# brown-ivl/manus

Hardware: AMD Instinct MI355X
Metric: train iters/sec (fwd+bwd) 300k Gaussians @1080p, 8 views; PSNR parity (higher is better)
Workload: dtype f32

## Files before the change

### include/manus_hip.h

```cpp
#ifndef MANUS_HIP_H
#define MANUS_HIP_H

#include <stddef.h>
#include <stdint.h>

#ifdef __cplusplus
extern "C" {
#endif

#define MGR_VERSION 100
#define MGR_CAM_FLOATS 40
#define MGR_TILE 16
#define MGR_MAX_BONES 32

enum {
    MGR_OK = 0,
    MGR_EINVAL = -1,
    MGR_ENOMEM = -2,
    MGR_EHIP = -3,
    MGR_EOVERFLOW = -4,
    MGR_ECUT = -6,
    MGR_ETIER = -7,
    MGR_ESTATE = -8
};
// ... 235 lines not shown
int mgr_fk_adam(int U, int J, const int32_t* frames_listed, const float* d_theta, float* theta, float* m, float* v,
                const float* mask, const float* lo, const float* hi, double lr_rot, double lr_trans, double beta1, double beta2,
                double eps, int step, void* stream);

#define MGR_FK_MAX_KEYPOINTS 64
size_t mgr_fk_terms_workspace_bytes(int U, int J, int K);
int mgr_fk_backward_terms(int V, int J, int F, int U, const int32_t* frames_listed, const int32_t* view_rows,
                          const int32_t* frame_of_view, const float* rest, const float* local, const int32_t* parents, const float* base,
                          const float* theta, const float* mask, const float* d_transforms, float* d_theta,
                          const float* theta_ref, const int32_t* neighbours,
                          double w_dev_rot, double w_smooth_rot, double w_dev_trans, double w_smooth_trans,
                          int K, const int32_t* kp_bone, const float* kp_offset, const float* kp_target, const float* kp_weight, double w_kp,
                          double* values, void* workspace, size_t workspace_bytes, void* stream);

size_t mgr_fk_terms2d_workspace_bytes(int U, int J, int K, int C);
int mgr_fk_backward_terms2d(int V, int J, int F, int U, const int32_t* frames_listed, const int32_t* view_rows,
                            const int32_t* frame_of_view, const float* rest, const float* local, const int32_t* parents, const float* base,
                            const float* theta, const float* mask, const float* d_transforms, float* d_theta,
                            const float* theta_ref, const int32_t* neighbours,
                            double w_dev_rot, double w_smooth_rot, double w_dev_trans, double w_smooth_trans,
                            int K, const int32_t* kp_bone, const float* kp_offset, const float* kp_target, const float* kp_weight, double w_kp,
                            int C, const float* kp2d_proj, const float* kp2d_target, const float* kp2d_weight,
                            double w_kp2d, double delta, double z_min, float* kp2d_dist,
                            double* values, void* workspace, size_t workspace_bytes, void* stream);

#define MGR_TRI_MAX_CAMERAS 64
int mgr_triangulate(int F, int C, int K, const float* proj, const float* targets, const float* weights,
                    double tau, double min_conf, int min_views, double z_min, double det_min,
                    int refit_rounds, int gn_iters,
                    float* xyz, float* conf, int32_t* n_inliers, uint8_t* inliers, float* dist, void* stream);

int mgr_project_points(int N, const float* xyz, const float* K9, const float* E12, float* uv,
                       void* stream);

int mgr_dilate_mask(int H, int W, int kernel_size, const uint8_t* mask, uint8_t* scratch, uint8_t* out,
                    void* stream);
int mgr_points_outside_mask(int N, const float* xyz, const float* K9, const float* E12, int H, int W,
                            const uint8_t* mask, int n_keypoints, const float* keypoints, uint8_t* out,
                            void* stream);
int mgr_keypoint_far_mask(int N, const float* xyz, int n_keypoints, const float* keypoints, float thresh,
                          uint8_t* out, void* stream);

size_t mgr_knn3_workspace_bytes(int N);
int mgr_knn3_mean_dist2(int N, const float* xyz, float* out, void* workspace,
                        size_t workspace_bytes, void* stream);

#define MGR_KNN_MAX_K 512
#ifndef MGR_KNN_CELL_K_DIV
#define MGR_KNN_CELL_K_DIV 16.0f
#endif
#define MGR_KNN_CELL_MIN_POINTS 2.0f
size_t mgr_knn_self_workspace_bytes(int N, int k);
int mgr_knn_self(int N, const float* xyz, int k, int include_self, float* out_d2, int32_t* out_idx, float* out_sigma,
                 int32_t* out_count, void* workspace, size_t workspace_bytes, void* stream);

#define MGR_LOOP_LAMBDA 1.0f
#define MGR_LOOP_SQRT2 1.41421356237309505f
size_t mgr_outlier_scores_workspace_bytes(int N, int k);
int mgr_outlier_scores(int N, const float* xyz, int k, int include_self, float prob, float* out_score, uint8_t* out_mask,
                       float* out_sigma, float* out_plof, double* out_stats, void* workspace, size_t workspace_bytes,
                       void* stream);

int mgr_l1_loss_grad(int64_t count, const float* a, const float* b, float scale, float* dL_da,
                     float* loss_sum, void* stream);

size_t mgr_image_loss_workspace_bytes(int V, int H, int W);
int mgr_image_loss(int V, int H, int W, const float* pred, const float* target, float w_l1, float w_ssim,
                   float grad_scale, float loss_offset, float* dL_dpred, float* sums, void* workspace,
                   size_t workspace_bytes, void* stream);
int mgr_image_loss_tiles(int V, int H, int W, const float* pred, const float* target, const float* bg3,
                         const uint32_t* tile_start, float w_l1, float w_ssim, float grad_scale, float loss_offset,
                         float* dL_dpred, float* sums, void* workspace, size_t workspace_bytes, void* stream);
int mgr_image_loss_tiles_list(int V, int H, int W, const float* target, const float* bg3, const uint32_t* tile_start,
                              void* workspace, size_t workspace_bytes, void* stream);
size_t mgr_image_loss_target_map_words(int V, int H, int W);
int mgr_image_loss_target_map(int V, int H, int W, const float* target, const float* bg3, uint32_t* map, void* stream);
int mgr_image_loss_tiles_list_mapped(int V, int H, int W, const uint32_t* map, const float* bg3, const uint32_t* tile_start,
                                     void* workspace, size_t workspace_bytes, int workspace_kept, void* stream);
int mgr_views_forward_attach_loss_list(const void* raster_workspace, int V, int H, int W, const uint32_t* map,
                                       void* loss_workspace, size_t loss_workspace_bytes);
int mgr_image_loss_tiles_finish(int V, int H, int W, const float* pred, const float* target, float w_l1, float w_ssim,
                                float grad_scale, float loss_offset, float* dL_dpred, float* sums, void* workspace,
                                size_t workspace_bytes, void* stream);

#define MGR_IL2D_DENSE 1
size_t mgr_image_loss2d_workspace_bytes(int V, int H, int W);
int mgr_image_loss2d_block(void);
int mgr_image_loss2d(int V, int H, int W, const float* pred, const float* target, const float* mask, float w_l1, float w_ssim,
                     float grad_scale, float loss_offset, float* dL_dpred, float* sums, float* view_sums, int flags,
                     void* workspace, size_t workspace_bytes, void* stream);

size_t mgr_map_loss_workspace_bytes(int V, int H, int W);
int mgr_map_loss(int V, int H, int W, const float* alpha, const float* mask, const float* depth, const float* depth_target,
                 float w_mask, float w_depth, float grad_scale, float* dL_dalpha, float* dL_ddepth, float* sums,
                 void* workspace, size_t workspace_bytes, void* stream);

int mgr_exposure_block(void);
size_t mgr_exposure_workspace_bytes(int V, int H, int W);
int mgr_exposure_apply(int V, int H, int W, int C, const int32_t* cam_of_view, const float* E, const float* img, float* out,
                       void* stream);
int mgr_exposure_backward(int V, int H, int W, int C, const int32_t* cam_of_view, const float* E, const float* img,
                          const float* g_in, float* g_out, float* dE, void* workspace, size_t workspace_bytes, void* stream);
int mgr_exposure_adam(int C, int U, const int32_t* cams_listed, int V, const int32_t* cam_of_view, const float* dE, float* E,
                      float* m, float* v, double lr, double beta1, double beta2, double eps, int step, void* stream);

size_t mgr_lpips_net_bytes(int net);
int mgr_lpips_net_pack(int net, const float* const* conv_w, const float* const* conv_b, const float* const* lin_w, void* blob,
                       size_t blob_bytes, void* stream);
size_t mgr_lpips_workspace_bytes(int net, int H, int W, int need_grad);
int mgr_lpips_layout(int net, int H, int W, int need_grad, size_t* offsets, int n);
int mgr_lpips(int net, int V, int H, int W, const float* pred, const float* target, const float* mask, const void* blob,
              size_t blob_bytes, int normalize, float grad_scale, float* values, float* dL_dpred, int accumulate,
              void* workspace, size_t workspace_bytes, void* stream);
size_t mgr_lpips_conv_scratch_bytes(int Cin, int Cout, int KH, int KW);
int mgr_lpips_conv(int Cin, int Cout, int H, int W, int KH, int KW, int stride, int pad, const float* x, const float* gate,
                   const float* w, const float* bias, int relu, int transposed, float* y, void* scratch, size_t scratch_bytes,
                   void* stream);
enum { MGR_LPIPS_F32 = 0, MGR_LPIPS_BF16 = 1 };
size_t mgr_lpips_net_bytes_op(int net, int operands);
int mgr_lpips_net_pack_op(int net, const float* const* conv_w, const float* const* conv_b, const float* const* lin_w, void* blob,
                          size_t blob_bytes, void* stream, int operands);
int mgr_lpips_op(int net, int V, int H, int W, const float* pred, const float* target, const float* mask, const void* blob,
                 size_t blob_bytes, int normalize, float grad_scale, float* values, float* dL_dpred, int accumulate,
                 void* workspace, size_t workspace_bytes, void* stream, int operands);
size_t mgr_lpips_conv_scratch_bytes_op(int Cin, int Cout, int KH, int KW, int operands);
int mgr_lpips_conv_op(int Cin, int Cout, int H, int W, int KH, int KW, int stride, int pad, const float* x, const float* gate,
                      const float* w, const float* bias, int relu, int transposed, float* y, void* scratch, size_t scratch_bytes,
                      void* stream, int operands);

size_t mgr_lpips_roi_workspace_bytes(int net, int V, const int* rects, int need_grad);
size_t mgr_lpips_taps_bytes(int net, int h, int w);
int mgr_lpips_roi_taps_op(int net, int H, int W, const int* rect, const float* target_v, const float* mask_v, const void* blob,
                          size_t blob_bytes, int normalize, float* taps_out, void* workspace, size_t workspace_bytes, void* stream,
                          int operands);
int mgr_lpips_roi_op(int net, int V, int H, int W, const int* rects, const float* pred, const float* target, const float* mask,
                     const void* blob, size_t blob_bytes, int normalize, const float* grad_scales, float* values, float* dL_dpred,
                     int accumulate, const float* const* target_taps, void* workspace, size_t workspace_bytes, void* stream,
                     int operands);
int mgr_lpips_roi(int net, int V, int H, int W, const int* rects, const float* pred, const float* target, const float* mask,
                  const void* blob, size_t blob_bytes, int normalize, const float* grad_scales, float* values, float* dL_dpred,
                  int accumulate, const float* const* target_taps, void* workspace, size_t workspace_bytes, void* stream);

#define LP_MAX_BATCH 16
size_t mgr_lpips_roi_batch_workspace_bytes(int net, int V, const int* rects, int need_grad, int max_batch);
int mgr_lpips_roi_taps_batch_op(int net, int V, int H, int W, const int* rects, const float* target, const float* mask, const void* blob,
                                size_t blob_bytes, int normalize, float* const* taps_out, int max_batch, void* workspace,
                                size_t workspace_bytes, void* stream, int operands);
int mgr_lpips_roi_batch_op(int net, int V, int H, int W, const int* rects, const float* pred, const float* target, const float* mask,
                           const void* blob, size_t blob_bytes, int normalize, const float* grad_scales, float* values, float* dL_dpred,
                           int accumulate, const float* const* target_taps, void* workspace, size_t workspace_bytes, void* stream,
                           int operands, int max_batch);
int mgr_lpips_roi_batch(int net, int V, int H, int W, const int* rects, const float* pred, const float* target, const float* mask,
                        const void* blob, size_t blob_bytes, int normalize, const float* grad_scales, float* values, float* dL_dpred,
                        int accumulate, const float* const* target_taps, void* workspace, size_t workspace_bytes, void* stream,
                        int max_batch);

enum { MGR_LPIPS_STORE_F32 = 0, MGR_LPIPS_STORE_BF16 = 1 };
size_t mgr_lpips_workspace_bytes_st(int net, int H, int W, int need_grad, int storage);
int mgr_lpips_layout_st(int net, int H, int W, int need_grad, size_t* offsets, int n, int storage);
size_t mgr_lpips_taps_bytes_st(int net, int h, int w, int storage);
size_t mgr_lpips_roi_batch_workspace_bytes_st(int net, int V, const int* rects, int need_grad, int max_batch, int storage);
int mgr_lpips_st(int net, int V, int H, int W, const float* pred, const float* target, const float* mask, const void* blob,
                 size_t blob_bytes, int normalize, float grad_scale, float* values, float* dL_dpred, int accumulate, void* workspace,
                 size_t workspace_bytes, void* stream, int operands, int storage);
int mgr_lpips_roi_batch_st(int net, int V, int H, int W, const int* rects, const float* pred, const float* target, const float* mask,
                           const void* blob, size_t blob_bytes, int normalize, const float* grad_scales, float* values, float* dL_dpred,
// ... 105 lines not shown
```

### manus_amd/_lib.py

```python
import ctypes
import os

import weakref

import torch

_HERE = os.path.dirname(os.path.abspath(__file__))
_VARIANT = os.environ.get("MANUS_HIP_VARIANT", "")
LIB_PATH = os.path.join(_HERE, "libmanus_hip%s.so" % ("_" + _VARIANT if _VARIANT else ""))
_LIB = None

MGR_CAM_FLOATS = 40
MGR_MAX_BONES = 32
MGR_FK_MAX_KEYPOINTS = 64
MGR_TRI_MAX_CAMERAS = 64
MGR_FRAMES_MAX_VIEWS = 16

MGR_OK, MGR_EINVAL, MGR_ENOMEM, MGR_EHIP, MGR_EOVERFLOW, MGR_ECUT, MGR_ETIER, MGR_ESTATE = 0, -1, -2, -3, -4, -6, -7, -8
MGR_FWD_CHECK, MGR_FWD_NO_BLEND, MGR_FWD_BLEND_ONLY, MGR_FWD_DEPTH_CUT = 1, 2, 4, 8
MGR_FWD_SKIP_BOX_LARGE, MGR_FWD_SKIP_BOX_MID, MGR_FWD_SKIP_SORT_BEHIND, MGR_FWD_RANK_LARGE = 16, 32, 128, 256
MGR_FWD_IMAGE_KEPT, MGR_FWD_REPAIR, MGR_FWD_SPREAD = 1024, 2048, 4096
MGR_BWD_CHECK, MGR_BWD_OUTPUTS_KEPT = 1, 512
MGR_OVF_PAIRS, MGR_OVF_CUT, MGR_OVF_TIER, MGR_OVF_FLAGS_MASK, MGR_OVF_REPAIRED_SHIFT = 1, 2, 4, 0xFFFF, 16
MGR_TIERS_BOX_LARGE, MGR_TIERS_BOX_MID, MGR_TIERS_WIDE_RECT = 1, 2, 4
MGR_TIERS_NEAR_SMALL_SHIFT, MGR_TIERS_NEAR_LARGE_SHIFT, MGR_TIERS_NEAR_MASK = 8, 16, 0xFF
MGR_TIERS_BEYOND_SMALL_SHIFT, MGR_TIERS_BEYOND_SMALL_MASK = 24, 0x7F
MGR_LPIPS_F32, MGR_LPIPS_BF16 = 0, 1
MGR_LPIPS_STORE_F32, MGR_LPIPS_STORE_BF16 = 0, 1
MGR_IL2D_DENSE = 1
MGR_KNN_MAX_K = 512
LP_MAX_BATCH = 16

c_int, c_i64, c_f32, c_vp, c_sz = ctypes.c_int, ctypes.c_int64, ctypes.c_float, ctypes.c_void_p, ctypes.c_size_t


class MgrFrameView(ctypes.Structure):
    _fields_ = [("offset", ctypes.c_int64), ("x0", ctypes.c_int32), ("y0", ctypes.c_int32), ("x1", ctypes.c_int32), ("y1", ctypes.c_int32),
                ("rx0", ctypes.c_int32), ("ry0", ctypes.c_int32), ("rx1", ctypes.c_int32), ("ry1", ctypes.c_int32),
                ("bg", ctypes.c_float * 3), ("slot", ctypes.c_int32)]


SIGNATURES = {
    "mgr_version": (c_int, []),
    "mgr_build_variant": (c_int, []),
    "mgr_raster_repair_max_tiles": (c_int, []),
    "mgr_last_error": (ctypes.c_char_p, []),
    "mgr_raster_workspace_bytes": (c_sz, [c_int, c_int, c_int, c_int, c_i64]),
    "mgr_raster_forward": (c_int, [c_int, c_int, c_int, c_int, c_vp, c_vp, c_vp, c_i64, c_vp, c_i64, c_vp,
                                   c_i64, c_vp, c_i64, c_vp, c_vp, c_vp, c_sz, c_i64, c_int, c_vp]),
    "mgr_raster_backward": (c_int, [c_int, c_int, c_int, c_int, c_vp, c_vp, c_vp, c_i64, c_vp, c_i64, c_vp,
                                    c_i64, c_vp, c_i64, c_vp, c_vp, c_vp, c_vp, c_vp, c_vp, c_vp, c_vp, c_sz,
                                    c_i64, c_int, c_vp]),
    "mgr_raster_blend_features": (c_int, [c_int, c_int, c_int, c_int, c_int, c_vp, c_i64, c_vp, c_int, c_vp, c_vp, c_vp, c_sz,
                                          c_i64, c_vp]),
    "mgr_raster_feat_backward_workspace_bytes": (c_sz, [c_int, c_int, c_int, c_int, c_int, c_i64]),
    "mgr_raster_blend_features_backward": (c_int, [c_int] * 5 + [c_vp, c_vp, c_i64, c_vp, c_i64, c_vp, c_i64, c_vp, c_int] + [c_vp] * 9
                                           + [c_vp, c_sz, c_i64, c_vp, c_sz, c_int, c_vp]),
    "mgr_raster_forward_seq_sync": (c_int, [c_vp, ctypes.POINTER(ctypes.c_uint32), c_vp]),
    "mgr_sh_to_half": (c_int, [c_int, c_vp, c_vp, c_vp]),
    "mgr_views_forward": (c_int, [c_int] * 7 + [c_vp] * 12 + [c_vp, c_sz, c_i64, c_int, c_vp]),
    "mgr_views_backward": (c_int, [c_int] * 7 + [c_vp] * 13 + [c_f32] + [c_vp] * 10 + [c_vp, c_sz, c_i64, c_int, c_vp]),
    "mgr_views_pose_workspace_bytes": (c_sz, [c_int, c_int, c_int]),
    "mgr_views_backward_pose": (c_int, [c_int] * 7 + [c_vp] * 13 + [c_f32] + [c_vp] * 10 + [c_vp, c_sz, c_i64, c_int, c_vp, c_vp, c_sz,
                                        c_vp]),
    "mgr_views_maps_backward_workspace_bytes": (c_sz, [c_int, c_int, c_int, c_int, c_i64]),
    "mgr_views_maps_backward": (c_int, [c_int] * 6 + [c_vp] * 11 + [c_int] + [c_vp] * 5 + [c_vp, c_sz, c_i64, c_vp, c_sz, c_int, c_vp]),
    "mgr_views_maps_pose_workspace_bytes": (c_sz, [c_int, c_int, c_int]),
    "mgr_views_maps_backward_pose": (c_int, [c_int] * 6 + [c_vp] * 11 + [c_int] + [c_vp] * 5 + [c_vp, c_sz, c_i64, c_vp, c_sz, c_int] +
                                     [c_int, c_vp, c_vp, c_sz, c_vp]),
    "mgr_raster_record_bytes": (c_int, []),
    "mgr_raster_layout": (c_int, [c_int, c_int, c_int, c_int, c_i64, ctypes.POINTER(c_sz), c_int]),
    "mgr_raster_status_sync": (c_int, [c_vp, ctypes.POINTER(c_i64), ctypes.POINTER(ctypes.c_int32), c_vp]),
    "mgr_raster_set_status_mirror": (c_int, [c_vp, c_vp]),
    "mgr_raster_set_cut_margin": (c_int, [c_f32, c_int, c_f32, c_f32, c_int]),
    "mgr_raster_set_cut_penalty": (c_int, [c_int]),
    "mgr_raster_status_tiers_sync": (c_int, [c_vp, ctypes.POINTER(c_i64), ctypes.POINTER(ctypes.c_int32),
                                             ctypes.POINTER(ctypes.c_int32), c_vp]),
    "mgr_debug_pair_alpha": (c_int, [c_int, c_vp, c_vp, c_vp, c_vp, c_vp, c_vp]),
    "mgr_raster_debug_binning_sync": (c_int, [c_vp, c_int, c_int, c_int, c_int, c_i64, c_int, c_vp, c_vp,
                                              c_i64, c_vp]),
    "mgr_skin_weights_fwd": (c_int, [c_int, c_vp, c_vp, c_int, c_int, c_int, c_int, c_int, c_vp, c_vp, c_vp,
                                     c_vp]),
    "mgr_skin_weights_bwd": (c_int, [c_int, c_vp, c_vp, c_int, c_int, c_int, c_int, c_int, c_vp, c_vp, c_vp,
                                     c_vp, c_int, c_vp]),
    "mgr_skin_weights_bwd_indexed": (c_int, [c_int, c_vp, c_vp, c_int, c_int, c_int, c_int, c_int, c_vp, c_vp, c_vp,
                                             c_vp, c_vp, c_vp, c_int, c_vp]),
    "mgr_skin_grid_bwd_workspace_bytes": (c_sz, [c_int, c_int, c_int, c_int]),
    "mgr_skin_grid_bwd": (c_int, [c_int, c_vp, c_vp, c_int, c_int, c_int, c_int, c_int, c_vp, c_vp, c_vp, c_vp, c_vp, c_int,
                                  c_vp, c_vp, c_vp, c_int, c_vp, c_sz, c_vp]),
    "mgr_skin_grid_adam": (c_int, [c_vp, c_vp, c_vp, c_int, c_vp, c_int, c_int, c_vp, c_vp, ctypes.c_double, ctypes.c_double, ctypes.c_double,
                                   ctypes.c_double, c_int, c_int, c_f32, c_vp]),
    "mgr_skin_grid_refine_workspace_bytes": (c_sz, [c_int]),
    "mgr_skin_grid_refine": (c_int, [c_vp, c_vp, c_vp, c_int, c_vp, c_vp, c_int, c_int, c_vp, c_vp, ctypes.c_double, ctypes.c_double,
                                     ctypes.c_double, ctypes.c_double, c_int, c_int, c_f32, ctypes.c_double, c_int, c_f32, c_vp, c_vp,
                                     c_sz, c_vp]),
    "mgr_skin_rows_mask": (c_int, [c_int, c_int, c_vp, c_vp, c_vp]),
    "mgr_views_backward_run_lists": (c_int, [c_int]),
    "mgr_views_active_list": (c_int, [c_vp, c_int, c_int, c_int, c_int, c_i64, ctypes.POINTER(c_vp), ctypes.POINTER(c_vp)]),
    "mgr_lbs_cov_fwd": (c_int, [c_int, c_int, c_int, c_vp, c_vp, c_vp, c_vp, c_vp, c_vp, c_vp, c_vp, c_vp]),
    "mgr_lbs_cov_bwd": (c_int, [c_int, c_int, c_int, c_vp, c_vp, c_vp, c_vp, c_vp, c_vp, c_vp, c_vp, c_vp,
                                c_vp, c_vp, c_vp, c_vp]),
    "mgr_lbs_cov_fwd_rows": (c_int, [c_int, c_int, c_int, c_vp, c_vp, c_vp, c_vp, c_vp, c_vp, c_vp, c_vp, c_int, c_vp]),
    "mgr_lbs_cov_bwd_rows": (c_int, [c_int, c_int, c_int, c_vp, c_vp, c_vp, c_vp, c_vp, c_vp, c_vp, c_vp, c_int, c_vp,
                                     c_vp, c_vp, c_vp, c_vp]),
    "mgr_lbs_pose_workspace_bytes": (c_sz, [c_int, c_int, c_int]),
    "mgr_lbs_pose_bwd": (c_int, [c_int, c_int, c_int, c_vp, c_vp, c_vp, c_vp, c_vp, c_vp, c_vp, c_vp, c_int, c_vp, c_vp, c_sz, c_vp]),
    "mgr_sh_color_fwd_rows": (c_int, [c_int, c_int, c_vp, c_vp, c_i64, c_vp, c_i64, c_int, c_vp, c_vp, c_vp]),
    "mgr_sh_color_bwd_rows": (c_int, [c_int, c_int, c_vp, c_vp, c_i64, c_vp, c_i64, c_int, c_vp, c_vp, c_vp, c_vp, c_vp,
                                      c_vp]),
    "mgr_sh_color_fwd": (c_int, [c_int, c_int, c_vp, c_vp, c_i64, c_vp, c_i64, c_vp, c_vp, c_vp]),
    "mgr_sh_color_bwd": (c_int, [c_int, c_int, c_vp, c_vp, c_i64, c_vp, c_i64, c_vp, c_vp, c_vp, c_vp, c_vp,
                                 c_vp]),
    "mgr_pack_camera": (c_int, [c_f32, c_f32, c_vp, c_vp, c_vp, c_vp, c_vp]),
    "mgr_bone_transforms": (c_int, [c_int, c_int, c_vp, c_vp, c_vp, c_vp]),
    "mgr_pose_apply": (c_int, [c_int, c_int, c_int] + [c_vp] * 8 + [c_vp]),
    "mgr_pose_backward": (c_int, [c_int, c_int, c_int, c_int] + [c_vp] * 10 + [c_vp]),
    "mgr_pose_adam": (c_int, [c_int, c_int] + [c_vp] * 9 + [ctypes.c_double] * 5 + [c_int, c_vp]),
    "mgr_pose_prior_workspace_bytes": (c_sz, [c_int, c_int]),
    "mgr_pose_backward_prior": (c_int, [c_int, c_int, c_int, c_int] + [c_vp] * 10 + [c_vp] + [ctypes.c_double] * 4 + [c_vp, c_vp, c_sz, c_vp]),
    "mgr_fk_apply": (c_int, [c_int, c_int, c_int] + [c_vp] * 11 + [c_vp]),
    "mgr_fk_backward": (c_int, [c_int, c_int, c_int, c_int] + [c_vp] * 11 + [c_vp]),
    "mgr_fk_adam": (c_int, [c_int, c_int] + [c_vp] * 8 + [ctypes.c_double] * 5 + [c_int, c_vp]),
    "mgr_fk_terms_workspace_bytes": (c_sz, [c_int, c_int, c_int]),
    "mgr_fk_backward_terms": (c_int, [c_int, c_int, c_int, c_int] + [c_vp] * 11 + [c_vp, c_vp] + [ctypes.c_double] * 4
                              + [c_int] + [c_vp] * 4 + [ctypes.c_double] + [c_vp, c_vp, c_sz, c_vp]),
    "mgr_fk_terms2d_workspace_bytes": (c_sz, [c_int, c_int, c_int, c_int]),
    "mgr_fk_backward_terms2d": (c_int, [c_int, c_int, c_int, c_int] + [c_vp] * 11 + [c_vp, c_vp] + [ctypes.c_double] * 4
                                + [c_int] + [c_vp] * 4 + [ctypes.c_double] + [c_int] + [c_vp] * 3 + [ctypes.c_double] * 3 + [c_vp]
                                + [c_vp, c_vp, c_sz, c_vp]),
    "mgr_triangulate": (c_int, [c_int, c_int, c_int, c_vp, c_vp, c_vp, ctypes.c_double, ctypes.c_double, c_int, ctypes.c_double,
                                ctypes.c_double, c_int, c_int] + [c_vp] * 5 + [c_vp]),
    "mgr_project_points": (c_int, [c_int, c_vp, c_vp, c_vp, c_vp, c_vp]),
    "mgr_dilate_mask": (c_int, [c_int, c_int, c_int, c_vp, c_vp, c_vp, c_vp]),
    "mgr_points_outside_mask": (c_int, [c_int, c_vp, c_vp, c_vp, c_int, c_int, c_vp, c_int, c_vp, c_vp, c_vp]),
    "mgr_keypoint_far_mask": (c_int, [c_int, c_vp, c_int, c_vp, c_f32, c_vp, c_vp]),
    "mgr_knn3_workspace_bytes": (c_sz, [c_int]),
    "mgr_knn3_mean_dist2": (c_int, [c_int, c_vp, c_vp, c_vp, c_sz, c_vp]),
    "mgr_knn_self_workspace_bytes": (c_sz, [c_int, c_int]),
    "mgr_knn_self": (c_int, [c_int, c_vp, c_int, c_int, c_vp, c_vp, c_vp, c_vp, c_vp, c_sz, c_vp]),
    "mgr_outlier_scores_workspace_bytes": (c_sz, [c_int, c_int]),
    "mgr_outlier_scores": (c_int, [c_int, c_vp, c_int, c_int, c_f32, c_vp, c_vp, c_vp, c_vp, c_vp, c_vp, c_sz, c_vp]),
    "mgr_exchange_mask": (c_int, [c_int, c_vp, c_int, ctypes.POINTER(c_i64), ctypes.POINTER(c_int), c_i64, c_vp, c_vp, c_vp, c_vp]),
    "mgr_exchange_index_workspace_bytes": (c_sz, [c_int]),
    "mgr_exchange_index": (c_int, [c_int, c_vp, c_vp, c_vp, c_vp, c_sz, c_vp]),
    "mgr_exchange_pack": (c_int, [c_int, c_int, c_vp, c_vp, c_int, ctypes.POINTER(c_i64), ctypes.POINTER(c_int), c_i64, c_vp, c_vp]),
    "mgr_exchange_unpack": (c_int, [c_int, c_int, c_vp, c_vp, c_int, ctypes.POINTER(c_i64), ctypes.POINTER(c_int), c_i64, c_vp, c_vp,
                                    c_i64, c_vp]),
    "mgr_exchange_pack_rows": (c_int, [c_int, c_int, c_vp, c_vp, c_vp, c_int, ctypes.POINTER(c_i64), ctypes.POINTER(c_int), c_i64, c_vp, c_vp]),
    "mgr_exchange_unpack_rows": (c_int, [c_int, c_int, c_vp, c_vp, c_vp, c_int, ctypes.POINTER(c_i64), ctypes.POINTER(c_int), c_i64, c_vp, c_vp,
                                         c_i64, c_vp]),
    "mgr_l1_loss_grad": (c_int, [c_i64, c_vp, c_vp, c_f32, c_vp, c_vp, c_vp]),
    "mgr_image_loss_workspace_bytes": (c_sz, [c_int, c_int, c_int]),
    "mgr_image_loss": (c_int, [c_int, c_int, c_int, c_vp, c_vp, c_f32, c_f32, c_f32, c_f32, c_vp, c_vp, c_vp, c_sz, c_vp]),
    "mgr_image_loss_tiles": (c_int, [c_int, c_int, c_int, c_vp, c_vp, c_vp, c_vp, c_f32, c_f32, c_f32, c_f32, c_vp, c_vp, c_vp, c_sz,
                                     c_vp]),
    "mgr_image_loss_target_map_words": (c_sz, [c_int, c_int, c_int]),
# ... 216 lines not shown
```

### manus_amd/csrc/image_loss.hip

```cpp
#include "mgr_common.h"
#include "il_list.h"
#include <cstdlib>

#define IL_ACC_SLOTS 64
#define IL_NX (IL_ND + 2 * IL_H1)

struct IlWindow {
    float g[11];
};

typedef mgr_v2f v2f;
__device__ __forceinline__ v2f il_v2(float a) { v2f r = {a, a}; return r; }

__global__ __launch_bounds__(IL_T) void k_image_loss(int H, int W, const float* __restrict__ pred,
                                                     const float* __restrict__ target, IlWindow win, float w_l1,
                                                     float w_ssim, float grad_scale, float* __restrict__ dL_dpred,
                                                     float2* __restrict__ partial, const uint32_t* __restrict__ work_list,
                                                     const uint32_t* __restrict__ work_count, int gxb, int gyb,
                                                     unsigned long long* __restrict__ acc_slots, uint32_t nb, float sum_lim,
                                                     uint32_t* __restrict__ bad_flag) {
    __shared__ v2f s_mix[5][3][IL_NX];
    __shared__ float s_red[4];
    const int tid = threadIdx.x;
    const uint32_t n_work = min(*work_count, nb);
// ... 312 lines not shown
        if (!tile_start) return;
    }
    uint32_t my_rank[(ILS_MAXW / IL_W + ILS_T) / ILS_T];
    int nmine = 0;
    for (int b = tid; b < gxb; b += ILS_T, ++nmine) {
        const int lo = max(b * IL_W - 2 * IL_H1, 0), hi = min(b * IL_W + IL_ND, W);
        uint32_t any = ((s_cand[b >> 5] >> (b & 31)) & 1u) ? 0u : 1u;
        for (int k = lo >> 5; k <= (hi - 1) >> 5 && !any; ++k) {
            uint32_t m = s_diff[k];
            const int base = k << 5;
            if (lo > base) m &= ~0u << (lo - base);
            if (hi < base + 32) m &= ~0u >> (base + 32 - hi);
            any |= m;
        }
        my_rank[nmine] = any ? atomicAdd(&s_n, 1u) : 0xFFFFFFFFu;
        if (!any) {
            const uint32_t bid = ((uint32_t)v * gridDim.x + blockIdx.x) * (uint32_t)gxb + (uint32_t)b;
            const int wcnt = min((b + 1) * IL_W, W) - b * IL_W;
            partial[bid] = make_float2(0.f, (float)(wcnt * 3 * rows));
        }
    }
    __syncthreads();
    if (tid == 0 && s_n) s_base = atomicAdd(work_count, s_n);
    __syncthreads();
    nmine = 0;
    for (int b = tid; b < gxb; b += ILS_T, ++nmine)
        if (my_rank[nmine] != 0xFFFFFFFFu)
            work_list[s_base + my_rank[nmine]] = ((uint32_t)v * gridDim.x + blockIdx.x) * (uint32_t)gxb + (uint32_t)b;
}

__global__ __launch_bounds__(ILS_T) void k_image_loss_list_mapped(IlListArgs a) {
    __shared__ uint32_t s2[2];
    il_list_mapped_block(a, (int)blockIdx.x, (int)blockIdx.y, s2);
}

__global__ __launch_bounds__(IL_ACC_SLOTS) void k_image_loss_fold(unsigned long long* __restrict__ acc_slots, long long total_px3,
                                                                  float* __restrict__ sums, float ca, float cb, float cc,
                                                                  uint32_t* __restrict__ work_count) {
    __shared__ unsigned long long s_fin[3 * IL_ACC_SLOTS];
    const int tid = threadIdx.x;
#pragma unroll
    for (int q = 0; q < 3; ++q) {
        s_fin[q * IL_ACC_SLOTS + tid] = acc_slots[3 * tid + q];
        acc_slots[3 * tid + q] = 0ull;
    }
    __syncthreads();
    if (tid == 0) {
        long long t_l1 = 0, t_ss = 0;
        unsigned long long t_px = 0;
        for (int k = 0; k < IL_ACC_SLOTS; ++k) {
            t_l1 += (long long)s_fin[k];
            t_ss += (long long)s_fin[IL_ACC_SLOTS + k];
            t_px += s_fin[2 * IL_ACC_SLOTS + k];
        }
        const double ta = (double)t_l1 * (1.0 / 4294967296.0);
        const double tb = (double)t_ss * (1.0 / 4294967296.0) + (double)((unsigned long long)total_px3 - t_px);
        const bool bad = work_count[1] != 0u;
        const float qnan = __int_as_float(0x7FC00000);
        sums[0] = bad ? qnan : (float)ta;
        sums[1] = bad ? qnan : (float)tb;
        sums[2] = bad ? qnan : (float)((double)ca * ta + (double)cb * tb + (double)cc);
        work_count[0] = 0u;
        work_count[1] = 0u;
    }
}


static size_t il_slots_offset(int64_t nb) { return (((size_t)nb * (sizeof(float2) + sizeof(uint32_t)) + 256) + 63) & ~(size_t)63; }
extern "C" size_t mgr_image_loss_workspace_bytes(int V, int H, int W) {
    if (V <= 0 || H <= 0 || W <= 0) return 0;
    return il_slots_offset(il_blocks(V, H, W)) + 3 * IL_ACC_SLOTS * sizeof(unsigned long long);
}

static int image_loss_impl(int V, int H, int W, const float* pred, const float* target, const float* bg3,
                           const uint32_t* tile_start, float w_l1, float w_ssim, float grad_scale, float loss_offset,
                           float* dL_dpred, float* sums, void* workspace, size_t workspace_bytes, void* stream_, int phase = 0,
                           const uint32_t* tmap = nullptr, bool clean = false) {
    if (V <= 0 || H <= 0 || W <= 0) return mgr_fail(MGR_EINVAL, "mgr_image_loss: bad sizes");
    if ((!target && !(phase == 1 && tmap)) || !workspace || (phase != 1 && (!pred || !dL_dpred || !sums))) return mgr_fail(MGR_EINVAL, "mgr_image_loss: null pointer");
    if (H > 65535 || V > 65535) return mgr_fail(MGR_EINVAL, "mgr_image_loss: H and V must fit a grid dimension");
    if (workspace_bytes < mgr_image_loss_workspace_bytes(V, H, W))
        return mgr_fail(MGR_ENOMEM, "mgr_image_loss: workspace too small");
    hipStream_t stream = (hipStream_t)stream_;
    IlWindow win;
    float sum = 0.f;
    for (int i = 0; i < 11; ++i) {
        win.g[i] = (float)exp(-(double)((i - 5) * (i - 5)) / (2.0 * 1.5 * 1.5));
        sum += win.g[i];
    }
    for (int i = 0; i < 11; ++i) win.g[i] /= sum;
    const dim3 grid((W + IL_W - 1) / IL_W, (H + 1) / 2, V);
    const int64_t nb = il_blocks(V, H, W);
    if (nb >= (1ll << 32)) return mgr_fail(MGR_EINVAL, "mgr_image_loss: image batch too large");
    float2* partial = (float2*)workspace;
    uint32_t* work_list = (uint32_t*)((char*)workspace + (size_t)nb * sizeof(float2));
    uint32_t* work_count = (uint32_t*)((char*)workspace + (size_t)nb * (sizeof(float2) + sizeof(uint32_t)) + 64);
    if (W > ILS_MAXW) return mgr_fail(MGR_EINVAL, "mgr_image_loss: image wider than 16384");
    unsigned long long* acc_slots = (unsigned long long*)((char*)workspace + il_slots_offset(nb));
    if (phase != 2 && !clean)
        MGR_HIP(hipMemsetAsync(work_count, 0, (size_t)((char*)(acc_slots + 3 * IL_ACC_SLOTS) - (char*)work_count), stream));
    if (phase == 2) {
    } else if (tile_start && tmap) {
        MGR_PROF("k_image_loss_list", stream);
        const IlListArgs la = il_list_args(V, H, W, tmap, tile_start, workspace);
        hipLaunchKernelGGL(k_image_loss_list_mapped, dim3((unsigned)la.nbx, V), dim3(ILS_T), 0, stream, la);
    } else if (tile_start) {
        MGR_PROF("k_image_loss_list", stream);
        hipLaunchKernelGGL(k_image_loss_list, dim3(grid.y, V), dim3(ILS_T), 0, stream, H, W, (int)grid.x, target, bg3, tile_start,
                           partial, work_list, work_count, tmap, (uint32_t*)nullptr);
    } else {
        MGR_PROF("k_image_loss_scan", stream);
        hipLaunchKernelGGL(k_image_loss_scan, dim3(grid.y, V), dim3(ILS_T), 0, stream, H, W, (int)grid.x, pred, target, dL_dpred,
                           partial, work_list, work_count);
    }
    if (phase == 1) return MGR_OK;
    {
        MGR_PROF("k_image_loss", stream);
#ifndef IL_GRID
#define IL_GRID (256 * 5)
#endif
        const int64_t pb = nb < IL_GRID ? nb : IL_GRID;
        const float sum_lim = (float)(2147483648.0 * (1.0 - 1.0 / 1048576.0) / (double)nb);
        hipLaunchKernelGGL(k_image_loss, dim3((unsigned)pb), dim3(IL_T), 0, stream, H, W, pred, target, win, w_l1, w_ssim,
                           grad_scale, dL_dpred, partial, (const uint32_t*)work_list, (const uint32_t*)work_count,
                           (int)grid.x, (int)grid.y, acc_slots, (uint32_t)nb, sum_lim, work_count + 1);
    }
    hipLaunchKernelGGL(k_image_loss_fold, dim3(1), dim3(IL_ACC_SLOTS), 0, stream, acc_slots, (long long)V * H * W * 3,
                       sums, grad_scale * w_l1, -grad_scale * w_ssim, loss_offset, work_count);
    MGR_LAUNCH_CHECK("k_image_loss", stream, 0);
    return MGR_OK;
}

extern "C" int mgr_image_loss(int V, int H, int W, const float* pred, const float* target, float w_l1, float w_ssim,
                              float grad_scale, float loss_offset, float* dL_dpred, float* sums, void* workspace,
                              size_t workspace_bytes, void* stream_) {
    return image_loss_impl(V, H, W, pred, target, nullptr, nullptr, w_l1, w_ssim, grad_scale, loss_offset, dL_dpred, sums,
                           workspace, workspace_bytes, stream_);
}

extern "C" int mgr_image_loss_tiles(int V, int H, int W, const float* pred, const float* target, const float* bg3,
                                    const uint32_t* tile_start, float w_l1, float w_ssim, float grad_scale, float loss_offset,
                                    float* dL_dpred, float* sums, void* workspace, size_t workspace_bytes, void* stream_) {
    if (!bg3 || !tile_start) return mgr_fail(MGR_EINVAL, "mgr_image_loss_tiles: null pointer");
    return image_loss_impl(V, H, W, pred, target, bg3, tile_start, w_l1, w_ssim, grad_scale, loss_offset, dL_dpred, sums,
                           workspace, workspace_bytes, stream_);
}

extern "C" int mgr_image_loss_tiles_list(int V, int H, int W, const float* target, const float* bg3, const uint32_t* tile_start,
                                         void* workspace, size_t workspace_bytes, void* stream_) {
    if (!bg3 || !tile_start) return mgr_fail(MGR_EINVAL, "mgr_image_loss_tiles_list: null pointer");
    return image_loss_impl(V, H, W, nullptr, target, bg3, tile_start, 0.f, 0.f, 0.f, 0.f, nullptr, nullptr, workspace,
                           workspace_bytes, stream_, 1);
}

extern "C" int mgr_image_loss_tiles_finish(int V, int H, int W, const float* pred, const float* target, float w_l1, float w_ssim,
                                           float grad_scale, float loss_offset, float* dL_dpred, float* sums, void* workspace,
                                           size_t workspace_bytes, void* stream_) {
    return image_loss_impl(V, H, W, pred, target, nullptr, nullptr, w_l1, w_ssim, grad_scale, loss_offset, dL_dpred, sums,
                           workspace, workspace_bytes, stream_, 2);
}

extern "C" size_t mgr_image_loss_target_map_words(int V, int H, int W) {
    if (V <= 0 || H <= 0 || W <= 0) return 0;
    return (size_t)V * ((H + 1) / 2) * ((W + 31) / 32);
}

extern "C" int mgr_image_loss_target_map(int V, int H, int W, const float* target, const float* bg3, uint32_t* map, void* stream_) {
    if (V <= 0 || H <= 0 || W <= 0) return mgr_fail(MGR_EINVAL, "mgr_image_loss_target_map: bad sizes");
    if (!target || !bg3 || !map) return mgr_fail(MGR_EINVAL, "mgr_image_loss_target_map: null pointer");
    if (H > 65535 || V > 65535 || W > ILS_MAXW) return mgr_fail(MGR_EINVAL, "mgr_image_loss_target_map: image too large");
    hipLaunchKernelGGL(k_image_loss_list, dim3((H + 1) / 2, V), dim3(ILS_T), 0, (hipStream_t)stream_, H, W, (W + IL_W - 1) / IL_W,
                       target, bg3, (const uint32_t*)nullptr, (float2*)nullptr, (uint32_t*)nullptr, (uint32_t*)nullptr,
                       (const uint32_t*)nullptr, map);
    MGR_LAUNCH_CHECK("k_image_loss_list", (hipStream_t)stream_, 0);
    return MGR_OK;
}

extern "C" int mgr_image_loss_tiles_list_mapped(int V, int H, int W, const uint32_t* map, const float* bg3, const uint32_t* tile_start,
                                                void* workspace, size_t workspace_bytes, int workspace_kept, void* stream_) {
    if (!map || !bg3 || !tile_start) return mgr_fail(MGR_EINVAL, "mgr_image_loss_tiles_list_mapped: null pointer");
    return image_loss_impl(V, H, W, nullptr, nullptr, bg3, tile_start, 0.f, 0.f, 0.f, 0.f, nullptr, nullptr, workspace,
                           workspace_bytes, stream_, 1, map, workspace_kept != 0);
}
```

### manus_amd/csrc/mgr_common.h

```cpp
#pragma once
#include <hip/hip_runtime.h>
#include <stdint.h>
#include <stdio.h>
#include <string.h>

#include "../../include/manus_hip.h"

#define MGR_WAVE 64

extern thread_local char g_mgr_err[512];

static inline int mgr_fail(int code, const char* fmt, const char* a = "", const char* b = "") {
    snprintf(g_mgr_err, sizeof(g_mgr_err), fmt, a, b);
    return code;
}

#define MGR_HIP(call)                                                                      \
    do {                                                                                   \
        hipError_t e_ = (call);                                                            \
        if (e_ != hipSuccess) return mgr_fail(MGR_EHIP, "%s: %s", #call, hipGetErrorString(e_)); \
    } while (0)

#define MGR_LAUNCH_CHECK(name, stream, debug)                                              \
    do {                                                                                   \
        hipError_t e_ = hipGetLastError();                                                 \
        if (e_ != hipSuccess) return mgr_fail(MGR_EHIP, "launch %s: %s", name, hipGetErrorString(e_)); \
        if (debug) {                                                                       \
            e_ = hipStreamSynchronize(stream);                                             \
            if (e_ != hipSuccess) return mgr_fail(MGR_EHIP, "sync %s: %s", name, hipGetErrorString(e_)); \
        }                                                                                  \
    } while (0)

void mgr_prof_begin(const char* name, hipStream_t stream);
void mgr_prof_end(hipStream_t stream);
extern int g_mgr_prof_on;
bool mgr_prof_match(const char* name);
struct MgrProfScope {
    hipStream_t s;
    bool on;
    MgrProfScope(const char* name, hipStream_t stream) : s(stream), on(g_mgr_prof_on != 0 && mgr_prof_match(name)) {
        if (on) mgr_prof_begin(name, s);
    }
    ~MgrProfScope() {
        if (on) mgr_prof_end(s);
    }
};
#define MGR_PROF(name, stream) MgrProfScope mgr_prof_scope_(name, stream)

#define MGR_WHY_UNITS 1u
#define MGR_WHY_VIEW_TILES 2u
#define MGR_WHY_CAND 4u
#define MGR_WHY_LIST 8u
#define MGR_WHY_EMPTY 16u
#define MGR_WHY_WINDOW 32u
#define MGR_REP_CAND 8192
#define MGR_REP_TARGET 3072
#define MGR_REP_VIEW_TILES 256
#define MGR_REP_MAX_TILES 65536
struct __attribute__((aligned(16))) MgrRepUnit {
    uint32_t vt, quad, nlist, start;
    uint32_t ck0, done_lo, done_hi, ntail;
    uint32_t ov_start, ov_ck0, p0, ck_first;
    uint32_t beyond;
    uint32_t pad[3];
};
struct __attribute__((aligned(16))) MgrRepTile {
    uint32_t tile, unit, zc, zw;
};
struct MgrRepView {
    uint32_t n, x0, y0, x1, y1, pad[3];
    MgrRepTile t[MGR_REP_VIEW_TILES];
};
struct MgrRep {
    MgrRepUnit* unit;
    float4* state;
    uint32_t* last;
    uint32_t* cnt;
    uint32_t* tile_rep;
    unsigned long long* cand;
    MgrRepView* view;
    uint32_t max_units, list_cap, ck_cap, list_base, ck_base;
};
struct MgrHeader {
    uint32_t total_pairs;
    uint32_t overflow;
    uint32_t epoch;
    uint32_t queue_len;
    uint32_t queue_head;
    uint32_t queue_head2;
    uint32_t n_items;
    uint32_t item_head;
    uint32_t queue_small;
    uint32_t queue_head3;
    uint32_t n_active;
    uint32_t queue_len_i;
    uint32_t acc_pairs, acc_flags;
    uint32_t tiers;
    uint32_t sort_big;
    uint32_t n_runs[4];
    uint32_t bwd_seq, rows_seq, rows_pending;
    uint32_t rows_owner[2];
    uint32_t fwd_seq, img_seq, img_owner[2], img_bg[3];
    uint32_t n_rep_units, rep_list_used, rep_ck_used;
    uint32_t rep_why;
    MgrRep rep;
    uint32_t sort_huge;
    uint32_t sort_large;
    uint32_t sort_near_large;
    uint32_t feat_seq, feat_dims[5], feat_flags;
    uint32_t spare[45 - 7 - sizeof(MgrRep) / 4];
    uint32_t queue_giant;
    uint32_t n_groups;
    uint32_t split_head, group_head;
    uint32_t pad2[56 - 8 - 68 + 64 - 4];
    uint32_t qctr[16 * 64];
    uint32_t qctr_f[16 * 64];
};
#define MGR_NCTR 16
#define MGR_HOLE 0xFFFFFFFEu
#define MGR_FEAT_CUT 1u
struct MgrFeatStamp {
    uint32_t dims[5], flags;
};
#define MGR_SKIP_BOX_LARGE 1
#define MGR_SKIP_BOX_MID 2
#define MGR_SKIP_SORT_BEHIND 4
#define MGR_SKIP_RANK_LARGE 8

#ifndef MGR_GREC_BYTES
#define MGR_GREC_BYTES 64
// ... 428 lines not shown
```

### manus_amd/csrc/raster_bwd.hip

```cpp
#include <atomic>

#include "instance_math.h"

#ifdef MGR_STATS
__device__ unsigned long long g_stats[16];
extern "C" int mgr_debug_stats(unsigned long long* dst) {
    return (int)hipMemcpyFromSymbol(dst, HIP_SYMBOL(g_stats), sizeof(unsigned long long) * 16);
}
__device__ unsigned long long g_bhist[3][65];
extern "C" int mgr_debug_bhist(unsigned long long* dst) {
    return (int)hipMemcpyFromSymbol(dst, HIP_SYMBOL(g_bhist), sizeof(unsigned long long) * 3 * 65);
}
#define BH(r, c, v) do { const int c_ = (c); const unsigned long long v_ = (unsigned long long)(v); if (lane == 0) atomicAdd(&g_bhist[r][c_], v_); } while (0)
#define MGR_STAT(i, v) do { const unsigned long long v_ = (unsigned long long)(v); if (lane == 0) atomicAdd(&g_stats[i], v_); } while (0)
#else
#define MGR_STAT(i, v)
#endif

#ifdef BWD_PROF
__device__ unsigned long long g_bprof[8];
extern "C" int mgr_debug_bprof(unsigned long long* dst) {
    return (int)hipMemcpyFromSymbol(dst, HIP_SYMBOL(g_bprof), sizeof(unsigned long long) * 8);
}
#define BP(k) { const long long now_ = wall_clock64(); acc_[k] += now_ - tp_; tp_ = now_; }
// ... 983 lines not shown
    inst_bwd_body<2, BMAX, MIXED, SH_HALF, true, NVV, POSE>(blk, n2, active_list + 2 * (size_t)N, MGR_IB_ARGS, pose_valid);
}
template <int NVV, int BMAX, bool MIXED, bool SH_HALF>
__global__ __launch_bounds__(IB_THREADS) __attribute__((amdgpu_waves_per_eu(MGR_IB_WAVES, MGR_IB_WAVES))) void k_inst_bwd_runs(MGR_IB_PARAMS) {
    inst_bwd_runs<NVV, BMAX, MIXED, SH_HALF, false>(MGR_IB_ALL, nullptr);
}

template <int G, int BMAX, bool MIXED, bool SH_HALF>
__global__ __launch_bounds__(IB_THREADS) __attribute__((amdgpu_waves_per_eu(MGR_IB_WAVES, MGR_IB_WAVES))) void k_inst_bwd_pose(MGR_IB_PARAMS, unsigned char* __restrict__ pose_valid) {
    inst_bwd_body<G, BMAX, MIXED, SH_HALF, false, 8, true>((int)blockIdx.x, (int)hdr->n_active, active_list, MGR_IB_ARGS, pose_valid);
}
template <int NVV, int BMAX, bool MIXED, bool SH_HALF>
__global__ __launch_bounds__(IB_THREADS) __attribute__((amdgpu_waves_per_eu(MGR_IB_WAVES, MGR_IB_WAVES))) void k_inst_bwd_runs_pose(MGR_IB_PARAMS, unsigned char* __restrict__ pose_valid) {
    inst_bwd_runs<NVV, BMAX, MIXED, SH_HALF, true>(MGR_IB_ALL, pose_valid);
}

template <int NV>
__global__ __launch_bounds__(256) void k_pose_part_views(int n_art, int B, int n_chunks, const float4* __restrict__ iacc,
                                                         const unsigned char* __restrict__ valid,
                                                         const float* __restrict__ skin_w, float* __restrict__ part) {
    constexpr int IPB = 256 / NV;
    __shared__ float s_rec[256 * MGR_POSE_REC];
    __shared__ unsigned char s_lst[NV * 256];
    __shared__ int s_cnt[8], s_wc[8 * 4];
    const int tid = threadIdx.x, vl = tid & (NV - 1), il = tid / NV;
    float pacc[12];
#pragma unroll
    for (int k = 0; k < 12; ++k) pacc[k] = 0.f;
    for (int c = blockIdx.x; c < n_chunks; c += gridDim.x) {
        const int i = c * IPB + il;
        const bool on = i < n_art && valid[(size_t)i * NV + vl] != 0;
        if (on) {
            const float4* o = iacc + ((size_t)i * NV + vl) * 3;
            const float4 a = o[0], b = o[1], d = o[2];
            float* r = s_rec + tid * MGR_POSE_REC;
            r[0] = a.x; r[1] = a.y; r[2] = a.z; r[3] = a.w; r[4] = b.x; r[5] = b.y; r[6] = b.z; r[7] = b.w;
            r[8] = d.x; r[9] = d.y; r[10] = d.z; r[11] = d.w;
            r[12] = __int_as_float(i);
        }
        pose_wg_lists<256>(tid, NV, on ? vl : -1, s_lst, s_cnt, s_wc);
        pose_wg_accumulate<256>(tid, NV, B, s_rec, s_lst, s_cnt, skin_w, pacc);
        __syncthreads();
    }
    pose_wg_store<256>(tid, NV, B, s_rec, pacc, part + (size_t)blockIdx.x * NV * B * 12);
}

static std::atomic<int> g_inst_runs{[] { const char* e = getenv("MANUS_INST_RUNS"); return e ? atoi(e) : 1; }()};
extern "C" int mgr_views_backward_run_lists(int on) { return g_inst_runs.exchange(on); }

struct CanonGrads {
    int B, n_art, sh_half;
    const float *xyz, *log_scale, *rot, *op_logit, *f_dc, *f_rest, *skin_w, *transforms;
    const int32_t* radii;
    float grad2d_scale;
    float *d_xyz, *d_ls, *d_rot, *d_op, *d_fdc, *d_frest, *d_w, *st_grad2d, *st_vis;
    int32_t* st_radii;
    float *d_T, *pose_part;
};

static int pose_view_slots(int n_art, int Gv) {
    const int ipb = 256 / Gv, chunks = (n_art + ipb - 1) / ipb;
    return chunks < MGR_POSE_MAX_WG ? chunks : MGR_POSE_MAX_WG;
}
static size_t pose_part_bytes(int N, int B, int Gv) { return ((size_t)pose_view_slots(N, Gv) * Gv * B * 12 * sizeof(float) + 255) & ~(size_t)255; }
extern "C" size_t mgr_views_pose_workspace_bytes(int V, int N, int B) {
    if (V <= 0 || N <= 0 || B <= 0) return 0;
    const int Gv = V <= 1 ? 1 : V <= 2 ? 2 : V <= 4 ? 4 : 8;
    return pose_part_bytes(N, B, Gv) + (size_t)N * Gv;
}

static int raster_backward_impl(int V, int N, int W, int H, const float* cams, const float* bg,
                                   const float* means3D, int64_t s_means, const float* cov3D,
                                   int64_t s_cov, const float* colors, int64_t s_col,
                                   const float* opacity, int64_t s_op, const float* out_color,
                                   const float* dL_dcolor, float* dL_dmeans3D, float* dL_dmeans2D, float* dL_dcolors,
                                   float* dL_dopacity, float* dL_dcov3D, const CanonGrads* canon, void* workspace,
                                   size_t workspace_bytes, int64_t cap, int flags, void* stream_) {
    (void)colors; (void)s_col; (void)opacity; (void)s_op;
    hipStream_t stream = (hipStream_t)stream_;
    if (V <= 0 || N < 0 || W <= 0 || H <= 0 || cap < 0)
        return mgr_fail(MGR_EINVAL, "mgr_raster_backward: bad sizes");
    if (!cams || !bg || !dL_dcolor || !out_color || !workspace)
        return mgr_fail(MGR_EINVAL, "mgr_raster_backward: null pointer");
    if (N == 0) return MGR_OK;
    if (!canon && (!means3D || !cov3D || !dL_dmeans3D || !dL_dmeans2D || !dL_dcolors || !dL_dopacity || !dL_dcov3D))
        return mgr_fail(MGR_EINVAL, "mgr_raster_backward: null pointer");
    const int gx = (W + 15) / 16, gy = (H + 15) / 16;
    const MgrLayout L = mgr_layout(V, N, W, H, cap);
    if (workspace_bytes < L.total) return mgr_fail(MGR_ENOMEM, "mgr_raster_backward: workspace too small");
    char* ws = (char*)workspace;
    MgrHeader* hdr = (MgrHeader*)(ws + L.header);
    static std::atomic<uint32_t> g_epoch{0};
    uint32_t epoch = g_epoch.fetch_add(1) + 1;
    if (epoch == 0) epoch = g_epoch.fetch_add(1) + 1;

    { MGR_PROF("k_blend_bwd", stream); hipLaunchKernelGGL(k_blend_bwd, dim3(256 * BWD_WAVES), dim3(256), 0, stream, N, W, H, gx, gy,
                       (const uint32_t*)(ws + L.sorted_gid), (const MgrGRec*)(ws + L.grec), (const uint32_t*)(ws + L.n_contrib),
                       (const float4*)(ws + L.ckpt), (const uint4*)(ws + L.items), hdr, out_color,
                       dL_dcolor, (uint32_t*)(ws + L.pair_tag), (float4*)(ws + L.pair_grad),
                       (uint32_t*)(ws + L.inst_tag), (uint32_t)cap, epoch); }
    MGR_LAUNCH_CHECK("k_blend_bwd", stream, flags & MGR_BWD_CHECK);
    if (canon) {
        const int Gv = V <= 1 ? 1 : V <= 2 ? 2 : V <= 4 ? 4 : 8;
        const int ipb = 256 / Gv;
        const size_t lds = (size_t)Gv * (MGR_CAM_FLOATS + (canon->skin_w ? IB_TSTRIDE(canon->B) : 0)) * sizeof(float);
        float4* iacc = (float4*)(ws + L.inst_grad);
        uint32_t* alist = (uint32_t*)(ws + L.inst_grad + (size_t)N * Gv * 48);
        const int ipb2 = IB_THREADS / Gv;
        const bool mixed = canon->skin_w && canon->n_art < N;
        int rounds = (int)((long long)N / ((long long)ipb * 1024));
        rounds = rounds < 1 ? 1 : (rounds > IG_ROUNDS ? IG_ROUNDS : rounds);
        const dim3 grid((N + ipb2 - 1) / ipb2), grid_g((N + ipb * rounds - 1) / (ipb * rounds));
        for (int v0 = 0; v0 < V; v0 += Gv) {
            const int vc = V - v0 < Gv ? V - v0 : Gv;
            const int accm = v0 > 0 ? 1 : 0;
            if (v0 > 0) {
                MGR_HIP(hipMemsetAsync(&hdr->n_active, 0, 4, stream));
                MGR_HIP(hipMemsetAsync(&hdr->n_runs[0], 0, 12, stream));
            }
            const bool runs = g_inst_runs.load(std::memory_order_relaxed) != 0 && Gv >= 4 && canon->B <= 24 && N < (1 << 24);
            const int rounds_r = rounds < Gv ? rounds : Gv;
            const dim3 grid_gr((N + ipb * rounds_r - 1) / (ipb * rounds_r));
            uint32_t* rlist = alist + (size_t)N;
            unsigned char* row_state = V <= Gv ? (unsigned char*)(rlist + 3 * (size_t)N) : nullptr;
            const int kept = (flags & MGR_BWD_OUTPUTS_KEPT) && V <= Gv ? 1 : 0;
#define MGR_IG_LAUNCH(GG)                                                                                             \
    hipLaunchKernelGGL((k_inst_gather<GG>), grid_g, dim3(256), 0, stream, v0, vc, N, canon->B, canon->n_art, canon->radii, \
                       (const ushort4*)(ws + L.rect), (const uint32_t*)(ws + L.pair_off),                             \
                       (const uint32_t*)(ws + L.pair_tag), (const float4*)(ws + L.pair_grad),                        \
                       (const uint32_t*)(ws + L.inst_tag), (uint32_t)cap, epoch, accm, rounds, iacc, alist, hdr, canon->d_xyz, canon->d_ls, canon->d_rot, canon->d_op, canon->d_fdc,    \
                       canon->d_frest, canon->d_w, canon->st_grad2d, canon->st_vis, canon->st_radii, runs && GG == 8 ? rlist : (uint32_t*)nullptr)
#define MGR_IB_LAUNCH(GG, BB)                                                                                         \
    if (mixed && canon->sh_half) MGR_IB_LAUNCH2(GG, BB, true, true);                                                  \
    else if (mixed) MGR_IB_LAUNCH2(GG, BB, true, false);                                                              \
    else if (canon->sh_half) MGR_IB_LAUNCH2(GG, BB, false, true);                                                     \
    else MGR_IB_LAUNCH2(GG, BB, false, false)
#define MGR_IB_LAUNCH2(GG, BB, MX, HF)                                                                                \
    hipLaunchKernelGGL((k_inst_bwd<GG, BB, MX, HF>), grid, dim3(IB_THREADS), lds, stream, v0, vc, N, canon->B, canon->n_art, W, H, cams, canon->xyz, \
                       canon->log_scale, canon->rot, canon->op_logit, canon->f_dc, canon->f_rest, canon->skin_w,      \
                       canon->transforms, (const float4*)iacc, (const uint32_t*)alist, (const MgrHeader*)hdr,         \
                       canon->grad2d_scale, accm, canon->d_xyz, canon->d_ls, canon->d_rot, canon->d_op, canon->d_fdc, \
                       canon->d_frest, canon->d_w, canon->st_grad2d)
            {
                MGR_PROF("k_inst_gather", stream);
#define MGR_IGR_LAUNCH(GG)                                                                                            \
    hipLaunchKernelGGL((k_inst_gather_runs<GG>), grid_gr, dim3(256), 0, stream, v0, vc, N, canon->B, canon->n_art, canon->radii, \
                       (const ushort4*)(ws + L.rect), (const uint32_t*)(ws + L.pair_off),                             \
                       (const uint32_t*)(ws + L.pair_tag), (const float4*)(ws + L.pair_grad),                        \
                       (const uint32_t*)(ws + L.inst_tag), (uint32_t)cap, epoch, accm, rounds_r, iacc, alist, hdr, canon->d_xyz, canon->d_ls, canon->d_rot, canon->d_op, canon->d_fdc, \
                       canon->d_frest, canon->d_w, canon->st_grad2d, canon->st_vis, canon->st_radii, rlist, row_state, kept)
                const bool old_gather = g_inst_runs.load(std::memory_order_relaxed) == 2 && Gv == 8;
                if (runs && !old_gather) {
                    if (Gv == 8) MGR_IGR_LAUNCH(8);
                    else if (Gv == 4) MGR_IGR_LAUNCH(4);
                    else if (Gv == 2) MGR_IGR_LAUNCH(2);
                    else MGR_IGR_LAUNCH(1);
                }
#undef MGR_IGR_LAUNCH
                else if (Gv == 8) MGR_IG_LAUNCH(8);
                else if (Gv == 4) MGR_IG_LAUNCH(4);
                else if (Gv == 2) MGR_IG_LAUNCH(2);
                else MGR_IG_LAUNCH(1);
            }
            MgrProfScope prof_ib(canon->d_T ? "k_inst_bwd_pose" : "k_inst_bwd", stream);
#define MGR_IBR_LAUNCH(MX, HF)                                                                                        \
    if (Gv == 8) MGR_IBR_LAUNCH2(8, MX, HF); else if (Gv == 4) MGR_IBR_LAUNCH2(4, MX, HF); else MGR_IBR_LAUNCH2(2, MX, HF)
// ... 151 lines not shown
```

### manus_amd/csrc/raster_feat.hip

```cpp
#include "instance_math.h"

#define FEAT_MAX_C 32
#define FEAT_GRID 4096

struct FeatArgs {
    int N, W, H, gx, gy, VT;
    uint32_t n_queue, n_busy, cap;
    const uint32_t* tile_queue;
    const uint4* tile_qrec;
    const uint32_t* sorted_gid;
    const MgrGRec* grec;
    const float* depth;
    const float* feat;
    long long s_feat;
    int C, c0, nc;
    int with_z;
    const float* bg;
    float* out;
    int Cout;
    float* out_alpha;
};

template <int CG>
__global__ __launch_bounds__(256) void k_blend_feat(const FeatArgs a) {
// ... 59 lines not shown
                mgr_pair_store(pb, rank & 1, ra.x, ra.y, ra.z, ra.w, rb.x, rb.y, 0.f, 0.f, 0.f, 0u);
                float* fr = frow + rank * CG;
#pragma unroll
                for (int k = 0; k < CG; ++k) fr[k] = f[k];
                if ((cnt & 1) && rank == cnt - 1) {
                    mgr_pair_pad(pb);
#pragma unroll
                    for (int k = 0; k < CG; ++k) fr[CG + k] = 0.0f;
                }
            }
            {
                gid = min(gid_n, gid_max);
                ra = *(const float4*)(gv + gid);
                rb = *((const float4*)(gv + gid) + 1);
                gid_n = sg[min(off + 128u + lane, lastidx)];
            }
            __builtin_amdgcn_wave_barrier();
            const int npair = (cnt + 1) >> 1;
            for (int p = 0; p < npair; ++p) {
                const float4* pp = (const float4*)(slab + p * MGR_PAIR_FLOATS);
                const float4 R0 = pp[0], R1 = pp[1], R2 = pp[2];
                float fa[CG], fb[CG];
                const float* fp = frow + 2 * p * CG;
#pragma unroll
                for (int k = 0; k < CG; ++k) { fa[k] = fp[k]; fb[k] = fp[CG + k]; }
                mgr_v2f dx, dy, G, al;
                bool va, vb;
                mgr_pair_alpha(R0, R1, R2, fpx2, fpy2, dx, dy, G, al, va, vb);
                {
                    const float al_a = (va && !done) ? al.x : 0.0f;
                    const float testT = Tr * (1.0f - al_a);
                    const bool stop = testT < 0.0001f;
                    const float w = stop ? 0.0f : al_a * Tr;
#pragma unroll
                    for (int k = 0; k < CG; ++k) acc[k] += fa[k] * w;
                    Tr = stop ? Tr : testT;
                    done = done || stop;
                }
                {
                    const float al_b = (vb && !done) ? al.y : 0.0f;
                    const float testT = Tr * (1.0f - al_b);
                    const bool stop = testT < 0.0001f;
                    const float w = stop ? 0.0f : al_b * Tr;
#pragma unroll
                    for (int k = 0; k < CG; ++k) acc[k] += fb[k] * w;
                    Tr = stop ? Tr : testT;
                    done = done || stop;
                }
                if (__builtin_amdgcn_ballot_w64(!done) == 0ull) break;
            }
        }
        if (inside) {
            const size_t pix = (size_t)py * W + px;
            if (ns > 0) {
                float* o = a.out + ((size_t)v * a.Cout + a.c0) * P + pix;
#pragma unroll
                for (int k = 0; k < CG; ++k)
                    if (k < ns) o[(size_t)k * P] = acc[k] + Tr * bg_of(k);
            }
            if (a.out_alpha) a.out_alpha[(size_t)v * P + pix] = 1.0f - Tr;
        }
    }
    for (uint32_t q = a.n_busy + blockIdx.x; q < (uint32_t)a.VT; q += gridDim.x) {
        const uint32_t vt = a.tile_queue[q];
        if (vt >= (uint32_t)a.VT) continue;
        const int v = (int)(vt / (uint32_t)T), t = (int)(vt % (uint32_t)T);
        const int px = (t % gx) * 16 + (tid & 15), py = (t / gx) * 16 + (tid >> 4);
        if (px < W && py < H) {
            const size_t pix = (size_t)py * W + px;
            if (ns > 0) {
                float* o = a.out + ((size_t)v * a.Cout + a.c0) * P + pix;
#pragma unroll
                for (int k = 0; k < CG; ++k)
                    if (k < ns) o[(size_t)k * P] = bg_of(k);
            }
            if (a.out_alpha) a.out_alpha[(size_t)v * P + pix] = 0.0f;
        }
    }
}

static int feat_read_state(const char* who, const char* ws, const MgrLayout& L, int V, int N, int W, int H, int64_t cap, int VT,
                           hipStream_t stream, MgrHeader& h) {
    const size_t head_bytes = offsetof(MgrHeader, qctr);
    MGR_HIP(hipMemcpyAsync(&h, ws + L.header, head_bytes, hipMemcpyDeviceToHost, stream));
    MGR_HIP(hipStreamSynchronize(stream));
    if (h.fwd_seq == 0u) return mgr_fail(MGR_ESTATE, "%s: no forward has run on this workspace", who);
    if (h.feat_seq != h.fwd_seq)
        return mgr_fail(MGR_ESTATE, "%s: the last forward on this workspace did not run its blend (MGR_FWD_NO_BLEND)", who);
    if (h.feat_dims[0] != (uint32_t)V || h.feat_dims[1] != (uint32_t)N || h.feat_dims[2] != (uint32_t)W ||
        h.feat_dims[3] != (uint32_t)H || h.feat_dims[4] != (uint32_t)cap)
        return mgr_fail(MGR_ESTATE, "%s: the last forward on this workspace was made for another V, N, W, H or pair capacity", who);
    if (h.feat_flags & MGR_FEAT_CUT)
        return mgr_fail(MGR_ESTATE, "%s: the last forward applied the depth cut (MGR_FWD_DEPTH_CUT): its lists are cut short", who);
    if (h.overflow != 0u)
        return mgr_fail(MGR_ESTATE, "%s: the last forward raised an overflow bit: its lists are incomplete", who);
    if (h.queue_len > (uint32_t)VT || h.queue_len_i > (uint32_t)VT)
        return mgr_fail(MGR_ESTATE, "%s: the header's queue lengths do not fit these sizes", who);
    return MGR_OK;
}

extern "C" int mgr_raster_forward_seq_sync(const void* workspace, uint32_t* seq, void* stream_) {
    hipStream_t stream = (hipStream_t)stream_;
    if (!workspace || !seq) return mgr_fail(MGR_EINVAL, "mgr_raster_forward_seq_sync: null pointer");
    MGR_HIP(hipMemcpyAsync(seq, (const char*)workspace + offsetof(MgrHeader, fwd_seq), 4, hipMemcpyDeviceToHost, stream));
    MGR_HIP(hipStreamSynchronize(stream));
    return MGR_OK;
}

extern "C" int mgr_raster_blend_features(int V, int N, int C, int W, int H, const float* features, int64_t stride_features,
                                         const float* bg_feat, int with_depth, float* out_feat, float* out_alpha,
                                         const void* workspace, size_t workspace_bytes, int64_t cap, void* stream_) {
    hipStream_t stream = (hipStream_t)stream_;
    if (V <= 0 || N < 0 || W <= 0 || H <= 0 || cap < 0 || cap > 0xFFFFFFF0ll)
        return mgr_fail(MGR_EINVAL, "mgr_raster_blend_features: bad sizes");
    if (C < 0 || C > FEAT_MAX_C) return mgr_fail(MGR_EINVAL, "mgr_raster_blend_features: C must be 0 .. 32");
    const int Cout = C + (with_depth ? 1 : 0);
    if (Cout == 0 && !out_alpha) return mgr_fail(MGR_EINVAL, "mgr_raster_blend_features: nothing to render (C = 0, no depth, no alpha)");
    if (!workspace || (Cout > 0 && !out_feat) || (C > 0 && N > 0 && !features))
        return mgr_fail(MGR_EINVAL, "mgr_raster_blend_features: null pointer");
    if (stride_features != 0 && stride_features < (int64_t)N * C)
        return mgr_fail(MGR_EINVAL, "mgr_raster_blend_features: view stride of the features smaller than N * C");
    const int gx = (W + 15) / 16, gy = (H + 15) / 16;
    if (gx > 65535 || gy > 65535) return mgr_fail(MGR_EINVAL, "mgr_raster_blend_features: image too large");
    const MgrLayout L = mgr_layout(V, N, W, H, cap);
    if (workspace_bytes < L.total) return mgr_fail(MGR_ENOMEM, "mgr_raster_blend_features: workspace too small for these sizes");
    const char* ws = (const char*)workspace;
    MgrHeader h;
    const int VT = V * gx * gy;
    {
        const int rc = feat_read_state("mgr_raster_blend_features", ws, L, V, N, W, H, cap, VT, stream, h);
        if (rc != MGR_OK) return rc;
    }

    FeatArgs a;
    a.N = N; a.W = W; a.H = H; a.gx = gx; a.gy = gy; a.VT = VT;
    a.n_queue = h.queue_len_i; a.n_busy = h.queue_len; a.cap = (uint32_t)cap;
    a.tile_queue = (const uint32_t*)(ws + L.tile_queue);
    a.tile_qrec = (const uint4*)(ws + L.tile_qrec);
    a.sorted_gid = (const uint32_t*)(ws + L.sorted_gid);
    a.grec = (const MgrGRec*)(ws + L.grec);
    a.depth = (const float*)(ws + L.depth);
    a.feat = features; a.s_feat = (long long)stride_features; a.C = C;
    a.bg = bg_feat; a.out = out_feat; a.Cout = Cout;
    int c0 = 0;
    bool first = true;
    MGR_PROF("k_blend_feat", stream);
    do {
        const int rem = Cout - c0, g = rem > 4 ? 8 : (rem > 2 ? 4 : 2), n = rem < g ? rem : g;
        a.c0 = c0;
        a.with_z = (with_depth && c0 + n == Cout) ? 1 : 0;
        a.nc = n - a.with_z;
        a.out_alpha = first ? out_alpha : nullptr;
        if (g == 8) hipLaunchKernelGGL(k_blend_feat<8>, dim3(FEAT_GRID), dim3(256), 0, stream, a);
        else if (g == 4) hipLaunchKernelGGL(k_blend_feat<4>, dim3(FEAT_GRID), dim3(256), 0, stream, a);
        else hipLaunchKernelGGL(k_blend_feat<2>, dim3(FEAT_GRID), dim3(256), 0, stream, a);
        MGR_LAUNCH_CHECK("k_blend_feat", stream, 0);
        c0 += n;
        first = false;
    } while (c0 < Cout);
    return MGR_OK;
}

#define FEAT_REC 16
#define FEAT_GEO 8

struct FeatScratch {
    size_t tag, rec, geo, total;
};
static inline FeatScratch feat_scratch_layout(int V, int N, int64_t cap) {
    FeatScratch S;
    const size_t c = (size_t)(cap > 0 ? cap : 1), VN = (size_t)V * (size_t)(N > 0 ? N : 1);
    size_t o = 0;
    S.tag = o; o += mgr_align(c * 4);
    S.rec = o; o += mgr_align(c * FEAT_REC * 4);
    S.geo = o; o += mgr_align(VN * FEAT_GEO * 4);
    S.total = o;
    return S;
}

extern "C" size_t mgr_raster_feat_backward_workspace_bytes(int V, int N, int C, int W, int H, int64_t cap) {
    (void)C; (void)W; (void)H;
    if (V <= 0 || N < 0 || cap < 0) return 0;
    return feat_scratch_layout(V, N, cap).total;
}

struct FeatBwdArgs {
// ... 737 lines not shown
```

### manus_amd/csrc/raster_fwd.hip

```cpp
#include <atomic>
#include <mutex>

#include "instance_math.h"
#include "il_list.h"

#include <cstdlib>
#include <cstring>
#include <map>
#include <string>
#include <vector>

thread_local char g_mgr_err[512] = {0};

int g_mgr_prof_on = 0;
namespace {
struct ProfRec { const char* name; hipEvent_t a, b; };
std::vector<ProfRec> g_prof_recs;
std::vector<hipEvent_t> g_prof_pool;
hipEvent_t prof_event() {
    if (!g_prof_pool.empty()) { hipEvent_t e = g_prof_pool.back(); g_prof_pool.pop_back(); return e; }
    hipEvent_t e;
    if (hipEventCreate(&e) != hipSuccess) return nullptr;
    return e;
}
// ... 1272 lines not shown
#endif
        for (uint32_t p = 0; p < parts; ++p) {
            const uint32_t a = parts == 1u ? lo : st[b0 + p], n = (parts == 1u ? hi : st[b0 + p + 1]) - a;
            if (n == 0) continue;
            __syncthreads();
            if (n <= lds_keys) {
                lds_sort_emit(keys + a, n, s_keys, s_cnt, s_scan, tid, out + a);
            } else {
                uint32_t npad = 1;
                while (npad < n) npad <<= 1;
                bitonic_mirror(keys + a, n, npad, tid, RS_THREADS);
                for (uint32_t t = tid; t < n; t += RS_THREADS) out[a + t] = (uint32_t)keys[a + t];
            }
        }
#ifdef DBS_PROF
        if (tid == 0) {
            const long long t2 = wall_clock64();
            atomicAdd(&g_dbsprof[0], (unsigned long long)(t1 - t0));
            atomicAdd(&g_dbsprof[1], (unsigned long long)(t2 - t1));
            atomicAdd(&g_dbsprof[2], 1ull);
            atomicAdd(&g_dbsprof[3], (unsigned long long)(hi - lo));
            atomicAdd(&g_dbsprof[4], (unsigned long long)parts);
            atomicMax(&g_dbsprof[5], (unsigned long long)(t2 - t0));
            atomicMax(&g_dbsprof[6], (unsigned long long)(hi - lo));
            atomicMax(&g_dbsprof[7], (unsigned long long)(t2 - t_start));
            const uint32_t nk = hi - lo;
            atomicAdd(&g_dbsprof[nk <= 1024u ? 8 : nk <= 2048u ? 9 : nk <= 3072u ? 10 : nk <= 4096u ? 11 : 12], 1ull);
        }
#endif
    }
}

#define DBR_THREADS RS_THREADS
template <int CAP>
__global__ __launch_bounds__(DBR_THREADS) void k_dbin_rank(int N, int V, int items_per_view, const uint32_t* __restrict__ db_start,
                                                           const uint32_t* __restrict__ db_item, const unsigned long long* __restrict__ db_keys,
                                                           uint32_t* __restrict__ db_order, MgrHeader* hdr,
                                                           int no_launch_behind, BgFill fill, int n_sort_blocks) {
    constexpr uint32_t cap_keys = (uint32_t)CAP;
    if ((int)blockIdx.x >= n_sort_blocks) {
        bg_fill_block(fill, hdr, (int)blockIdx.x - n_sort_blocks, (int)gridDim.x - n_sort_blocks);
        return;
    }
    __shared__ __attribute__((aligned(16))) unsigned long long s_keys[CAP];
    __shared__ uint32_t s_cnt[RS_WAVES * 256];
    __shared__ uint32_t s_scan[32];
    const int tid = threadIdx.x;
    const int v = (int)blockIdx.x % V, it = (int)blockIdx.x / V;
    const uint32_t* const ent = db_item + ((size_t)v * items_per_view + it) * 2;
    const uint32_t e0 = ent[0], e1 = ent[1];
    if (e0 == 0u) return;
    const uint32_t* st = db_start + (size_t)v * (MGR_DB_BUCKETS + 1);
    const uint32_t lo = st[~e0], hi = st[e1], n = hi - lo;
    if (n > (uint32_t)MGR_DB_RANK_MAX * 13u / 16u && tid == 0) {
        atomicAdd(&hdr->sort_big, 1u);
        if (n > (uint32_t)MGR_DB_RANK_LARGE * 13u / 16u) atomicAdd(&hdr->sort_near_large, 1u);
        if (n > (uint32_t)MGR_DB_RANK_MAX) atomicAdd(&hdr->sort_large, 1u);
    }
    if (n > cap_keys) {
        if (tid == 0) {
            atomicAdd(&hdr->sort_huge, 1u);
            if (no_launch_behind) atomicOr(&hdr->overflow, MGR_OVF_TIER);
        }
        return;
    }
    lds_sort_emit(db_keys + (size_t)v * N + lo, n, s_keys, s_cnt, s_scan, tid, db_order + (size_t)v * N + lo);
}

#define BIN_SMALL_TILES 2048
__device__ __forceinline__ bool bin_mine(ushort4 box, bool small_variant) {
    const uint32_t tb = (uint32_t)box.z * (uint32_t)box.w;
    return tb > 0u && (tb <= (uint32_t)BIN_SMALL_TILES) == small_variant;
}

#define BCNT_THREADS 256
#define BCNT_PER (MGR_BIN_BLOCK / BCNT_THREADS)
template <bool SMALL>
__global__ __launch_bounds__(BCNT_THREADS) void k_bin_count(int N, int T, int nblk, int bb,
                                                            const uint32_t* __restrict__ db_nvis,
                                                            const ushort4* __restrict__ db_bbox,
                                                            const uint32_t* __restrict__ db_order,
                                                            const ushort4* __restrict__ rect,
                                                            const unsigned long long* __restrict__ alive,
                                                            uint4* __restrict__ db_rec, uint32_t* __restrict__ bin_mat, int xcd_order) {
    extern __shared__ uint32_t s_mem[];
    uint32_t* s_hist = s_mem;
    const int tid = threadIdx.x;
    int v = blockIdx.y, b = blockIdx.x;
    if (xcd_order) {
        const int q = blockIdx.x >> 3;
        v = (blockIdx.x & 7) + 8 * (q / nblk);
        b = q % nblk;
    }
    const ushort4 box = db_bbox[v];
    if (!bin_mine(box, SMALL)) return;
    const uint32_t nvis = db_nvis[v];
    if ((uint32_t)b * (uint32_t)bb >= nvis) return;
    const int TB = (int)box.z * (int)box.w, bw = box.z;
    uint32_t gid[BCNT_PER];
#pragma unroll
    for (int r = 0; r < BCNT_PER; ++r) {
        const uint32_t p = (uint32_t)b * (uint32_t)bb + r * BCNT_THREADS + tid;
        gid[r] = (r * BCNT_THREADS < bb && p < nvis) ? db_order[(size_t)v * N + p] : 0u;
    }
    ushort4 rc[BCNT_PER];
    unsigned long long am[BCNT_PER];
#pragma unroll
    for (int r = 0; r < BCNT_PER; ++r) {
        rc[r] = rect[(size_t)v * N + gid[r]];
        am[r] = alive[(size_t)v * N + gid[r]];
    }
    for (int k = tid; k < TB; k += BCNT_THREADS) s_hist[k] = 0;
    __syncthreads();
#pragma unroll
    for (int r = 0; r < BCNT_PER; ++r) {
        const uint32_t p = (uint32_t)b * (uint32_t)bb + r * BCNT_THREADS + tid;
        if (r * BCNT_THREADS < bb && p < nvis) {
            const uint32_t w = rc[r].z - rc[r].x, h = rc[r].w - rc[r].y;
            db_rec[(size_t)v * N + p] = make_uint4((uint32_t)rc[r].x | ((uint32_t)rc[r].y << 16), w | (h << 16), (uint32_t)am[r],
                                                   (uint32_t)(am[r] >> 32));
            const int org = ((int)rc[r].y - (int)box.y) * bw + (int)rc[r].x - (int)box.x;
            if (w * h <= 64u) {
                const float rw = __frcp_rn((float)max(w, 1u));
                unsigned long long m = am[r];
                while (m) {
                    const uint32_t k = (uint32_t)__builtin_ctzll(m);
                    m &= m - 1ull;
                    const uint32_t ty = (uint32_t)(((float)k + 0.5f) * rw), tx = k - ty * w;
                    atomicAdd(&s_hist[org + (int)ty * bw + (int)tx], 1u);
                }
            } else {
                for (uint32_t y = 0; y < h; ++y)
                    for (uint32_t x = 0; x < w; ++x) atomicAdd(&s_hist[org + (int)y * bw + (int)x], 1u);
            }
        }
    }
    __syncthreads();
    uint32_t* row = bin_mat + ((size_t)v * nblk + b) * T;
    for (int k = tid; k < TB; k += BCNT_THREADS) row[k] = s_hist[k];
}

#define BSCAN_COLS 32
#define BSCAN_SEGS 32
__global__ __launch_bounds__(BSCAN_COLS * BSCAN_SEGS) void k_bin_scan(int gx, int T, int nblk, int bb, const uint32_t* __restrict__ db_nvis,
                                                                      const ushort4* __restrict__ db_bbox,
                                                                      const uint32_t* __restrict__ tile_start,
                                                                      uint32_t* __restrict__ bin_mat) {
    __shared__ uint32_t s_part[BSCAN_SEGS][BSCAN_COLS];
    const int v = blockIdx.y, col = threadIdx.x & (BSCAN_COLS - 1), seg = threadIdx.x / BSCAN_COLS;
    const int k = blockIdx.x * BSCAN_COLS + col;
    const ushort4 box = db_bbox[v];
    const int TB = (int)box.z * (int)box.w;
    if (blockIdx.x * BSCAN_COLS >= TB) return;
    const bool on = k < TB;
    const int nb = (int)((db_nvis[v] + (uint32_t)bb - 1u) / (uint32_t)bb);
    const int per = (nb + BSCAN_SEGS - 1) / BSCAN_SEGS, b0 = min(seg * per, nb), b1 = min(b0 + per, nb);
    uint32_t* colp = bin_mat + (size_t)v * nblk * T + (on ? k : 0);
    uint32_t sum = 0;
    if (on) {
        int b = b0;
        for (; b + 8 <= b1; b += 8) {
            uint32_t c[8];
#pragma unroll
            for (int j = 0; j < 8; ++j) c[j] = colp[(size_t)(b + j) * T];
#pragma unroll
            for (int j = 0; j < 8; ++j) sum += c[j];
        }
        for (; b < b1; ++b) sum += colp[(size_t)b * T];
    }
// ... 974 lines not shown
        const float qx0 = (float)(bx * 16 + (int)(quad & 1u) * 8), qy0 = (float)(by * 16 + (int)(quad >> 1) * 8);
        const int pslot = (int)(quad << 6) | lane;
        const float4 st = rep.state[(size_t)uq * 64 + lane];
        float Tr = st.w, C2 = st.z;
        mgr_v2f C01 = {st.x, st.y};
        uint32_t last = rep.last[(size_t)uq * 64 + lane];
        const unsigned long long exec_m = __builtin_amdgcn_ballot_w64(true);
        unsigned long long done_m = ((unsigned long long)rq.done_hi << 32) | rq.done_lo;
        const MgrGRec* const gv = grec + (size_t)v * N;
        float* const slab = s_slab + wave * 32 * MGR_PAIR_FLOATS;
        if (pre == 0u && p0 != 0u && (((~done_m & exec_m) >> lane) & 1ull)) ckpt[(size_t)ov_ck0 * 256 + pslot] = make_float4(C01.x, C01.y, C2, Tr);
        uint32_t j = 0;
        while (j < n) {
            const uint32_t blen = min(n - j, (uint32_t)MGR_CHUNK - ((nl + j) % MGR_CHUNK));
            int bx0, by0, bx1, by1;
            if (!mgr_quad_bbox(~done_m & exec_m, bx0, by0, bx1, by1)) break;
            bool alive = false;
            MgrGRec r;
            if ((uint32_t)lane < blen) {
                r = gv[(uint32_t)s_keys[j + lane]];
                alive = !mgr_box_dead(r.x, r.y, r.ca, r.cb, r.cc, mgr_qmax(r.op), qx0 + (float)bx0, qy0 + (float)by0, qx0 + (float)bx1,
                                      qy0 + (float)by1);
            }
            const unsigned long long m = __ballot(alive);
            const int cnt = __popcll(m);
            if (alive) {
                const int rank = __popcll(m & lt);
                float* pb = slab + (rank >> 1) * MGR_PAIR_FLOATS;
                mgr_pair_store<true>(pb, rank & 1, r.x, r.y, r.ca, r.cb, r.cc, r.op, r.r, r.g, r.b, nl + j + (uint32_t)lane + 1u);
                if ((cnt & 1) && rank == cnt - 1) mgr_pair_pad<true>(pb);
            }
            __builtin_amdgcn_wave_barrier();
            const int npair = (cnt + 1) >> 1;
            for (int p = 0; p < npair; ++p) {
                const float4* pp = (const float4*)(slab + p * MGR_PAIR_FLOATS);
                const float4 R0 = pp[0], R1 = pp[1], R2 = pp[2], R3 = pp[3], R4 = pp[4];
                if (mgr_fwd_pair_step(R0, R1, R2, R3, R4, fpx2, fpy2, Tr, C01, C2, last, done_m, exec_m)) break;
            }
            __builtin_amdgcn_wave_barrier();
            const uint32_t nextpos = nl + j + blen;
            if ((nextpos % MGR_CHUNK) == 0u && nextpos < total && (((~done_m & exec_m) >> lane) & 1ull))
                ckpt[(size_t)(ov_ck0 + nextpos / MGR_CHUNK - c0) * 256 + pslot] = make_float4(C01.x, C01.y, C2, Tr);
            j += blen;
        }
        if (inside) {
            const size_t pix = (size_t)py * W + px;
            n_contrib[(size_t)v * P + pix] = last;
            float* o = out_color + (size_t)v * 3 * P + pix;
            o[0] = C01.x + Tr * bg0;
            o[P] = C01.y + Tr * bg1;
            o[2 * P] = C2 + Tr * bg2;
        }
        const uint32_t mx = mgr_wave_max_u32(last);
        if (lane == 0) {
            tile_qdone[(size_t)vt * 4 + quad] = mx;
            if ((~done_m & exec_m) != 0ull && ru.beyond != 0u) { atomicOr(&hdr->acc_flags, MGR_OVF_CUT); atomicOr(&hdr->rep_why, MGR_WHY_WINDOW); }
        }
    }
}

static thread_local float g_cut_frac = 0.125f, g_cut_range = 0.0625f, g_cut_rel = 2.0e-4f;
static thread_local int g_cut_min = 64, g_cut_interior = 0, g_cut_penalty = 16;
extern "C" int mgr_raster_set_cut_penalty(int forwards) {
    if (forwards < 0 || forwards > 0x7FFFFFF) return mgr_fail(MGR_EINVAL, "mgr_raster_set_cut_penalty: 0 .. 2^27 forwards");
    g_cut_penalty = forwards;
    return MGR_OK;
}
extern "C" int mgr_raster_set_cut_margin(float frac_entries, int min_entries, float depth_range_frac, float depth_rel,
                                         int interior_only) {
    if (!(frac_entries >= 0.f) || min_entries < 0 || !(depth_range_frac >= 0.f) || !(depth_rel >= 0.f))
        return mgr_fail(MGR_EINVAL, "mgr_raster_set_cut_margin: margins must be non-negative");
    g_cut_frac = frac_entries; g_cut_min = min_entries; g_cut_range = depth_range_frac; g_cut_rel = depth_rel;
    g_cut_interior = interior_only ? 1 : 0;
    return MGR_OK;
}
__global__ __launch_bounds__(256) void k_fwd_items(const uint4* __restrict__ tile_qrec, const uint32_t* __restrict__ tile_qdone,
                                                   uint32_t* __restrict__ tile_done, uint4* __restrict__ items, MgrHeader* hdr,
                                                   int N, int T, const uint32_t* __restrict__ sorted_gid, const float* __restrict__ depth,
                                                   const uint32_t* __restrict__ tile_zused, const uint32_t* __restrict__ tile_qend,
                                                   uint32_t* __restrict__ tile_zcut, uint32_t* mirror, float cut_frac, uint32_t cut_min,
                                                   float cut_range, float cut_rel, int gx, int interior_only,
                                                   const uint32_t* __restrict__ tile_queue, int VT, unsigned char* __restrict__ tile_bgok,
                                                   const float* out_color, const float* __restrict__ bg, const MgrRep rep, uint32_t cut_penalty,
                                                   uint32_t* __restrict__ tile_zwin, const IlListArgs ll, int n_item_blocks, const MgrFeatStamp stamp) {
    __shared__ uint32_t s_scan[8];
    if ((int)blockIdx.x >= n_item_blocks) {
        const int lb = (int)blockIdx.x - n_item_blocks;
        il_list_mapped_block(ll, lb % ll.nbx, lb / ll.nbx, s_scan);
        return;
    }
    __shared__ uint32_t s_base;
    __shared__ uint32_t s_run[257];
    __shared__ uint4 s_qr[256], s_qd[256], s_rp[256];
    const int tid = threadIdx.x;
    const uint32_t n_busy = hdr->queue_len_i;
    const uint32_t nb = (n_busy + 255u) / 256u;
    if ((int)blockIdx.x == n_item_blocks - 1 && tid == 0) {
        const uint32_t f = hdr->acc_flags;
        uint32_t ovf = hdr->overflow;
        if (f) { ovf |= f; hdr->overflow = ovf; hdr->acc_flags = 0u; }
        if (mirror) {
            mirror[0] = hdr->total_pairs; mirror[1] = ovf | (min(hdr->n_rep_units, 0xFFFFu) << 16); mirror[2] = hdr->tiers | (min(hdr->sort_big, 0xFFu) << 8) | (min(hdr->sort_near_large, 0xFFu) << 16) | (min(hdr->sort_large, 0x7Fu) << 24);
            __threadfence_system();
            mirror[3] = 1u;
        }
    }
    for (uint32_t q = hdr->queue_len + blockIdx.x * 256u + (uint32_t)tid; q < (uint32_t)VT; q += (uint32_t)n_item_blocks * 256u) tile_bgok[tile_queue[q]] = 1;
    if (blockIdx.x == 0 && tid == 0) {
        const unsigned long long owner = (unsigned long long)(uintptr_t)out_color;
        hdr->img_seq = hdr->fwd_seq;
        hdr->img_owner[0] = (uint32_t)owner; hdr->img_owner[1] = (uint32_t)(owner >> 32);
        hdr->img_bg[0] = __float_as_uint(bg[0]); hdr->img_bg[1] = __float_as_uint(bg[1]); hdr->img_bg[2] = __float_as_uint(bg[2]);
        hdr->feat_seq = hdr->fwd_seq;
        for (int k = 0; k < 5; ++k) hdr->feat_dims[k] = stamp.dims[k];
        hdr->feat_flags = stamp.flags;
    }
    if (blockIdx.x >= nb) return;
    const uint32_t q = (uint32_t)tid * nb + blockIdx.x;
    uint4 qr = make_uint4(0, 0, 0, 0), qd = make_uint4(0, 0, 0, 0), rp = make_uint4(0, 0, 0, 0);
    uint32_t nch = 0;
    if (q < n_busy && tile_qrec[q].x != MGR_HOLE) {
        qr = tile_qrec[q];
        qd = *(const uint4*)(tile_qdone + (size_t)qr.x * 4);
        if (rep.max_units) {
            const uint32_t ro = rep.tile_rep[qr.x];
            if (ro != 0u) {
                const MgrRepUnit ru = rep.unit[ro - 1u];
                if (ru.ntail != 0u) rp = make_uint4(ru.p0 | 0x80000000u, ru.ov_start, ru.ov_ck0, ru.ck_first);
            }
        }
        const uint32_t tmax = max(max(qd.x, qd.y), max(qd.z, qd.w));
        tile_done[qr.x] = tmax;
        nch = (tmax + MGR_CHUNK - 1) / MGR_CHUNK;
        const uint32_t e = tile_qend[qr.x], nl = qr.z, used = tile_zused[qr.x];
        uint32_t hint = 0u;
        const uint32_t em = e + max(cut_min, (uint32_t)(cut_frac * (float)e));
        bool interior = e != 0xFFFFFFFFu && e > 0u;
        if (interior && interior_only) {
            const uint32_t t = qr.x % (uint32_t)T, vbase = qr.x - t;
            const int tx = (int)(t % (uint32_t)gx), ty = (int)(t / (uint32_t)gx), gy = T / gx;
            for (int dy = -1; dy <= 1; ++dy)
                for (int dx = -1; dx <= 1; ++dx) {
                    const int x = tx + dx, y = ty + dy;
                    if ((dx | dy) == 0 || x < 0 || y < 0 || x >= gx || y >= gy) continue;
                    const uint32_t q2 = tile_qend[vbase + (uint32_t)(y * gx + x)];
                    interior = interior && q2 != 0xFFFFFFFFu && q2 != 0u;
                }
        }
        const uint32_t pen = tile_zcut[qr.x];
        const bool ran_out = used != 0u && e == 0xFFFFFFFFu;
        if (ran_out) hint = cut_penalty;
        else if (pen > 1u) hint = pen - 1u;
        else if (interior && e <= nl && (em <= nl || used != 0u)) {
            const uint32_t* sg = sorted_gid + qr.y;
            const float* dv = depth + (size_t)(qr.x / (uint32_t)T) * N;
            const uint32_t g0 = sg[0], ge = sg[e - 1u], gm = sg[min(em, nl) - 1u];
            const float z0 = dv[g0], ze = dv[ge], zm = dv[gm];
            float zc = ze + cut_range * (ze - z0) + cut_rel * ze;
            const float zx = fmaxf(__uint_as_float(~used), ze + 1.5f * (float)(em - e) * (ze - z0) / (float)e);
            zc = fmaxf(zc, em <= nl ? zm : zx);
            hint = ~__float_as_uint(zc);
            if (used == 0u) {
                const uint32_t iw = max(em, e) + (uint32_t)MGR_REP_TARGET;
                tile_zwin[qr.x] = iw >= nl ? 0x7F7FFFFFu : __float_as_uint(fmaxf(dv[sg[iw - 1u]], zc));
            }
        }
        tile_zcut[qr.x] = hint;
    }
    uint32_t total;
    const uint32_t run = block_excl_scan(nch, s_scan, total);
    s_run[tid] = run;
    s_qr[tid] = qr;
    s_qd[tid] = qd;
    s_rp[tid] = rp;
    if (tid == 0) {
        s_run[256] = total;
        s_base = total ? atomicAdd(&hdr->n_items, total) : 0u;
    }
    __syncthreads();
    const uint32_t base = s_base;
    for (uint32_t i = (uint32_t)tid; i < total; i += 256u) {
        int lo = 0, hi = 256;
        while (hi - lo > 1) {
            const int mid = (lo + hi) >> 1;
            if (s_run[mid] <= i) lo = mid; else hi = mid;
        }
        const uint32_t c = i - s_run[lo];
        const uint4 r = s_qr[lo], x = s_rp[lo];
        uint32_t off = r.y + c * MGR_CHUNK, ck = r.w + (c > 0 ? c - 1 : 0);
        const uint32_t p0 = x.x & 0x7FFFFFFFu;
        if (x.x != 0u && c * MGR_CHUNK >= p0) {
            off = x.y + (c * MGR_CHUNK - p0);
            ck = c * MGR_CHUNK == p0 ? x.w : x.z + (c - p0 / MGR_CHUNK);
        }
        items[2 * (size_t)(base + i)] = make_uint4(r.x, c, off, ck);
        items[2 * (size_t)(base + i) + 1] = s_qd[lo];
    }
}

struct CanonInputs {
    int B, n_art, sh_half;
    const float *xyz, *log_scale, *rot, *op_logit, *f_dc, *f_rest, *skin_w, *transforms;
};

struct MgrSideStream {
    hipStream_t stream = nullptr;
    hipEvent_t fork = nullptr, join = nullptr;
    hipError_t init() {
        if (stream) return hipSuccess;
        hipError_t e = hipStreamCreateWithFlags(&stream, hipStreamNonBlocking);
        if (e != hipSuccess) return e;
        e = hipEventCreateWithFlags(&fork, hipEventDisableTiming);
        if (e != hipSuccess) return e;
        return hipEventCreateWithFlags(&join, hipEventDisableTiming);
    }
};
#define MGR_MAX_DEVICES 64
static MgrSideStream& mgr_side_stream(int device) {
    static thread_local MgrSideStream s[MGR_MAX_DEVICES];
    return s[device];
}

static std::mutex g_slot_mu;
template <typename T>
struct MgrSlots {
    struct { const void* ws; T v; } slot[64];
    bool set(const void* workspace, const T* v) {
        std::lock_guard<std::mutex> lk(g_slot_mu);
        int k_free = -1;
        for (int k = 0; k < 64; ++k) {
            if (slot[k].ws == workspace) { k_free = k; break; }
            if (!slot[k].ws && k_free < 0) k_free = k;
        }
        if (k_free < 0) return false;
        if (v) { slot[k_free].ws = workspace; slot[k_free].v = *v; }
        else if (slot[k_free].ws == workspace) slot[k_free].ws = nullptr;
        return true;
    }
    T take(const void* workspace) {
        std::lock_guard<std::mutex> lk(g_slot_mu);
        for (auto& m : slot)
            if (m.ws == workspace) { m.ws = nullptr; return m.v; }
        return T();
    }
};
static MgrSlots<uint32_t*> g_mirror;
static MgrSlots<IlListArgs> g_loss_list;

extern "C" int mgr_views_forward_attach_loss_list(const void* workspace, int V, int H, int W, const uint32_t* target_map,
                                                  void* loss_workspace, size_t loss_workspace_bytes) {
    if (!workspace) return mgr_fail(MGR_EINVAL, "mgr_views_forward_attach_loss_list: null workspace");
    if (!target_map) { g_loss_list.set(workspace, nullptr); return MGR_OK; }
    if (V <= 0 || H <= 0 || W <= 0 || W > ILS_MAXW || !loss_workspace) return mgr_fail(MGR_EINVAL, "mgr_views_forward_attach_loss_list: bad arguments");
    if (loss_workspace_bytes < (size_t)il_blocks(V, H, W) * 12 + 256) return mgr_fail(MGR_ENOMEM, "mgr_views_forward_attach_loss_list: loss workspace too small");
    const IlListArgs a = il_list_args(V, H, W, target_map, nullptr, loss_workspace);
    if (!g_loss_list.set(workspace, &a)) return mgr_fail(MGR_ENOMEM, "mgr_views_forward_attach_loss_list: too many pending lists");
    return MGR_OK;
}

extern "C" int mgr_raster_set_status_mirror(const void* workspace, void* host_words) {
    if (!workspace) return mgr_fail(MGR_EINVAL, "mgr_raster_set_status_mirror: null workspace");
    void* dev = nullptr;
    if (host_words) MGR_HIP(hipHostGetDevicePointer(&dev, host_words, 0));
    uint32_t* const words = (uint32_t*)dev;
    if (!g_mirror.set(workspace, host_words ? &words : nullptr))
        return mgr_fail(MGR_EINVAL, "mgr_raster_set_status_mirror: too many workspaces with a pending mirror");
    return MGR_OK;
}

static int raster_forward_impl(int V, int N, int W, int H, const float* cams, const float* bg,
                               const float* means3D, int64_t s_means, const float* cov3D,
                               int64_t s_cov, const float* colors, int64_t s_col,
                               const float* opacity, int64_t s_op, const CanonInputs* canon, float* out_color,
                               int32_t* radii, void* workspace, size_t workspace_bytes,
                               int64_t cap, int flags, void* stream_) {
    hipStream_t stream = (hipStream_t)stream_;
    const bool do_bin = !(flags & MGR_FWD_BLEND_ONLY), do_blend = !(flags & MGR_FWD_NO_BLEND), use_cut = (flags & MGR_FWD_DEPTH_CUT) && canon != nullptr;
    static const bool bg_fill_on = [] { const char* e = getenv("MANUS_BG_FILL"); return !(e && e[0] == 'b'); }();
    bool bg_filled = false;
    const int skip_tiers = ((flags & MGR_FWD_SKIP_BOX_LARGE) ? MGR_SKIP_BOX_LARGE : 0) | ((flags & MGR_FWD_SKIP_BOX_MID) ? MGR_SKIP_BOX_MID : 0) |
                           ((flags & MGR_FWD_SKIP_SORT_BEHIND) ? MGR_SKIP_SORT_BEHIND : 0) | ((flags & MGR_FWD_RANK_LARGE) ? MGR_SKIP_RANK_LARGE : 0);
    const int img_kept = (flags & MGR_FWD_IMAGE_KEPT) ? 1 : 0;
    const bool spread = (flags & MGR_FWD_SPREAD) != 0;
    const bool repair = use_cut && (flags & MGR_FWD_REPAIR) && W < 65536 && H < 65536 &&
                        (int64_t)((W + 15) / 16) * ((H + 15) / 16) <= (int64_t)MGR_REP_MAX_TILES;
    const int debug = flags & MGR_FWD_CHECK;
    if (V <= 0 || N < 0 || W <= 0 || H <= 0 || cap < 0 || cap > 0xFFFFFFF0ll)
        return mgr_fail(MGR_EINVAL, "mgr_raster_forward: bad sizes");
    if (!cams || !bg || !out_color || !workspace ||
        (N > 0 && !canon && (!means3D || !cov3D || !colors || !opacity)) || (N > 0 && !radii))
        return mgr_fail(MGR_EINVAL, "mgr_raster_forward: null pointer");
    const int gx = (W + 15) / 16, gy = (H + 15) / 16, T = gx * gy;
    if (gx > 65535 || gy > 65535) return mgr_fail(MGR_EINVAL, "mgr_raster_forward: image too large");
    const MgrLayout L = mgr_layout(V, N, W, H, cap);
    if (workspace_bytes < L.total) return mgr_fail(MGR_ENOMEM, "mgr_raster_forward: workspace too small");
    char* ws = (char*)workspace;
    MgrHeader* hdr = (MgrHeader*)(ws + L.header);
    uint32_t* tile_count = (uint32_t*)(ws + L.tile_count);
    uint32_t* tile_start = (uint32_t*)(ws + L.tile_start);
    const int VT = V * T;
    MgrRep rep_all;
    rep_all.unit = (MgrRepUnit*)(ws + L.rep_unit); rep_all.state = (float4*)(ws + L.rep_state); rep_all.last = (uint32_t*)(ws + L.rep_last);
    rep_all.cnt = (uint32_t*)(ws + L.rep_cnt); rep_all.tile_rep = (uint32_t*)(ws + L.tile_rep); rep_all.cand = (unsigned long long*)(ws + L.rep_cand);
    rep_all.view = (MgrRepView*)(ws + L.rep_view);
    rep_all.max_units = repair ? mgr_rep_units(cap) : 0u;
    rep_all.list_cap = mgr_rep_list(cap); rep_all.ck_cap = mgr_rep_ck(cap);
    rep_all.list_base = (uint32_t)cap; rep_all.ck_base = (uint32_t)(cap / MGR_CHUNK + 1);

    static std::atomic<bool> attr_set[MGR_MAX_DEVICES];
    int device = 0;
    MGR_HIP(hipGetDevice(&device));
    if (device < 0 || device >= MGR_MAX_DEVICES) return mgr_fail(MGR_EINVAL, "mgr_raster_forward: device index out of range");
    if (!attr_set[device].load(std::memory_order_acquire)) {
        MGR_HIP(hipFuncSetAttribute((const void*)k_tile_sort, hipFuncAttributeMaxDynamicSharedMemorySize,
                                    SORT_LDS_KEYS * 8 + RS_WAVES * 256 * 4 + 256));
        MGR_HIP(hipFuncSetAttribute((const void*)k_preprocess, hipFuncAttributeMaxDynamicSharedMemorySize,
                                    152 * 1024));
        MGR_HIP(hipFuncSetAttribute((const void*)k_emit, hipFuncAttributeMaxDynamicSharedMemorySize,
                                    152 * 1024));
        MGR_HIP(hipFuncSetAttribute((const void*)k_inst_fwd<false, false>, hipFuncAttributeMaxDynamicSharedMemorySize, 152 * 1024));
        MGR_HIP(hipFuncSetAttribute((const void*)k_inst_fwd<true, false>, hipFuncAttributeMaxDynamicSharedMemorySize, 152 * 1024));
        MGR_HIP(hipFuncSetAttribute((const void*)k_inst_fwd<false, true>, hipFuncAttributeMaxDynamicSharedMemorySize, 152 * 1024));
        MGR_HIP(hipFuncSetAttribute((const void*)k_inst_fwd<true, true>, hipFuncAttributeMaxDynamicSharedMemorySize, 152 * 1024));
        MGR_HIP(hipFuncSetAttribute((const void*)k_dbin_sort<SORT_LDS_KEYS>, hipFuncAttributeMaxDynamicSharedMemorySize,
                                    SORT_LDS_KEYS * 8 + RS_WAVES * 256 * 4 + 256));
        MGR_HIP(hipFuncSetAttribute((const void*)k_bin_count<false>, hipFuncAttributeMaxDynamicSharedMemorySize, 152 * 1024));
        MGR_HIP(hipFuncSetAttribute((const void*)k_bin_scatter<0, false>, hipFuncAttributeMaxDynamicSharedMemorySize, 152 * 1024));
        MGR_HIP(hipFuncSetAttribute((const void*)k_bin_scatter<0, true>, hipFuncAttributeMaxDynamicSharedMemorySize, 152 * 1024));
        MGR_HIP(hipFuncSetAttribute((const void*)k_repair_blend, hipFuncAttributeMaxDynamicSharedMemorySize, REP_BLEND_LDS));
        attr_set[device].store(true, std::memory_order_release);
    }

    const int lds_hist = ((size_t)T * 4 + 128 <= 150 * 1024) ? 1 : 0;
    const char* binning_env = getenv("MGR_BINNING");
    const bool ordered_env = !(binning_env && strcmp(binning_env, "sorted") == 0);
    const bool ordered = ordered_env && lds_hist && T <= 65535 && (size_t)T * 4 + BIN_SC_FIXED_BYTES <= 150 * 1024;
    const size_t hist_bytes = lds_hist ? (size_t)T * 4 : 0;
    if (do_bin) {

    if (N > 0) {
        dim3 grid((N + PRE_THREADS - 1) / PRE_THREADS, V);
        if (canon) {
            MGR_PROF("k_inst_fwd", stream);
            const bool mixed = canon->skin_w && canon->n_art < N;
#define MGR_IF_LAUNCH(MX, HF)                                                                                           \
    hipLaunchKernelGGL((k_inst_fwd<MX, HF>), dim3(8 * ((grid.x + 7) / 8) * V), dim3(PRE_THREADS), 128 + hist_bytes, stream, N, canon->B, canon->n_art, W, H, \
                       gx, gy, cams, canon->xyz, canon->log_scale, canon->rot, canon->op_logit, canon->f_dc,            \
                       canon->f_rest, canon->skin_w, canon->transforms, (MgrGRec*)(ws + L.grec),                        \
                       (float*)(ws + L.depth), (ushort4*)(ws + L.rect), (unsigned long long*)(ws + L.alive),            \
                       (uint32_t*)(ws + L.pair_off), tile_count, radii, hdr, lds_hist, V,                                  \
                       use_cut ? (const uint32_t*)(ws + L.tile_zcut) : (const uint32_t*)nullptr, (uint32_t*)(ws + L.db_zrange))
            if (mixed && canon->sh_half) MGR_IF_LAUNCH(true, true);
            else if (mixed) MGR_IF_LAUNCH(true, false);
            else if (canon->sh_half) MGR_IF_LAUNCH(false, true);
            else MGR_IF_LAUNCH(false, false);
#undef MGR_IF_LAUNCH
        } else
        { MGR_PROF("k_preprocess", stream); hipLaunchKernelGGL(k_preprocess, grid, dim3(PRE_THREADS), 128 + hist_bytes, stream, N, W, H, gx,
                           gy, cams, means3D, s_means, cov3D, s_cov, colors, s_col, opacity, s_op,
                           (MgrGRec*)(ws + L.grec), (float*)(ws + L.depth), (ushort4*)(ws + L.rect),
                           (unsigned long long*)(ws + L.alive), (uint32_t*)(ws + L.pair_off), tile_count, radii,
                           hdr, lds_hist, (uint32_t*)(ws + L.db_zrange)); }
        MGR_LAUNCH_CHECK("k_preprocess", stream, debug);
    }
    {
        const int nbT = (T + 1023) / 1024, nblk = V * nbT;
        uint2* part = (uint2*)(ws + L.scan_part);
        uint32_t* blk_cls = (uint32_t*)(ws + L.scan_cls);
        const int use_hint = ordered ? 1 : 0;
        const bool dbin = ordered && N > 0;
        const int n_bx = (N + 1024 * DB_PER - 1) / (1024 * DB_PER);
        uint4* blk_box = (uint4*)(ws + L.scan_box);
        const DbinArgs dba = {N, n_bx, (const int32_t*)radii, (const float*)(ws + L.depth), (const ushort4*)(ws + L.rect),
                              (const unsigned long long*)(ws + L.alive), dbin ? (uint32_t*)(ws + L.db_count) : nullptr,
                              (uint32_t*)(ws + L.db_cursor), (uint32_t*)(ws + L.db_start), (uint32_t*)(ws + L.db_nvis),
                              (ushort4*)(ws + L.db_bbox), (unsigned long long*)(ws + L.db_keys), (uint32_t*)(ws + L.db_zrange),
                              (uint32_t*)(ws + L.db_item), (N + MGR_DB_ITEM - 1) / MGR_DB_ITEM + 1, (N + PRE_THREADS - 1) / PRE_THREADS};
        { MGR_PROF("k_tile_scan_a", stream); hipLaunchKernelGGL(k_tile_scan_a, dim3(nblk + (dbin ? n_bx * V : 0)), dim3(1024), 0, stream, T, nbT, tile_count,
                           (const uint32_t*)(ws + L.tile_done), use_hint, part, blk_cls, blk_box, gx, nblk, dba, hdr); }
        { MGR_PROF("k_tile_scan_b", stream); hipLaunchKernelGGL(k_tile_scan_b, dim3(nblk + (dbin ? V : 0)), dim3(1024), 0, stream, V, T, nbT, tile_count, part, (const uint32_t*)blk_cls,
                           tile_start, (uint32_t*)(ws + L.tile_cursor), (uint32_t*)(ws + L.tile_queue), (uint4*)(ws + L.tile_qrec),
                           (const uint32_t*)(ws + L.tile_done), use_hint, (uint32_t*)(ws + L.chunk_start), hdr, (uint32_t)cap,
                           (uint32_t*)(ws + L.tile_zcut), (uint32_t*)(ws + L.tile_zused), (uint32_t*)(ws + L.tile_qend), use_cut ? 1 : 0, (const uint4*)blk_box, dba, (unsigned char*)(ws + L.tile_bgok), (uint32_t*)(ws + L.tile_rep), rep_all); }
    }
    MGR_LAUNCH_CHECK("k_tile_scan", stream, debug);
    if (N > 0 && ordered) {
        const int bb = mgr_bin_block(V, N), nblk = (N + bb - 1) / bb;
        const ushort4* rect = (const ushort4*)(ws + L.rect);
        const unsigned long long* alive = (const unsigned long long*)(ws + L.alive);
        uint32_t* db_start = (uint32_t*)(ws + L.db_start);
        uint32_t* db_nvis = (uint32_t*)(ws + L.db_nvis);
        unsigned long long* db_keys = (unsigned long long*)(ws + L.db_keys);
        uint32_t* db_order = (uint32_t*)(ws + L.db_order);
        uint32_t* bin_mat = (uint32_t*)(ws + L.bin_mat);
        uint4* db_rec = (uint4*)(ws + L.db_rec);
        ushort4* db_bbox = (ushort4*)(ws + L.db_bbox);
        const dim3 grid_n((N + 1024 * DB_PER - 1) / (1024 * DB_PER), V), grid_b(nblk, V);
        const int chunk = bb == MGR_BIN_BLOCK ? DB_CHUNK : 1024, chunks = (N + chunk - 1) / chunk;
        const size_t rec_bytes = BIN_SC_FIXED_BYTES;
        { MGR_PROF("k_dbin_scatter", stream); hipLaunchKernelGGL(k_dbin_scatter, grid_n, dim3(1024), 0, stream, N, (const int32_t*)radii, (const float*)(ws + L.depth), rect, alive,
                           (const uint32_t*)db_start, (uint32_t*)(ws + L.db_cursor), db_keys, (const uint32_t*)(ws + L.db_zrange), (N + PRE_THREADS - 1) / PRE_THREADS); }
        { MGR_PROF("k_dbin_sort", stream);
          const int ipv = (N + MGR_DB_ITEM - 1) / MGR_DB_ITEM + 1;
          const bool ranked = ipv <= DBR_MAX_ITEMS;
          const bool behind = !ranked || !(skip_tiers & MGR_SKIP_SORT_BEHIND);
          BgFill fill = {do_blend && bg_fill_on ? out_color : nullptr, (const uint32_t*)(ws + L.tile_queue), bg, VT, T, gx, W, H,
                         (const unsigned char*)(ws + L.tile_bgok), img_kept};
          const BgFill none = {nullptr, nullptr, nullptr, 0, 0, 0, 0, 0, nullptr, 0};
          const int n_fill = fill.out ? 1024 : 0;
          bg_filled = fill.out != nullptr;
          const uint32_t cap_keys = (skip_tiers & MGR_SKIP_RANK_LARGE) ? (uint32_t)MGR_DB_RANK_LARGE : (uint32_t)MGR_DB_RANK_MAX;
          if (ranked && (skip_tiers & MGR_SKIP_RANK_LARGE))
              hipLaunchKernelGGL((k_dbin_rank<MGR_DB_RANK_LARGE>), dim3((unsigned)(ipv * V + n_fill)), dim3(DBR_THREADS), 0, stream, N, V, ipv, (const uint32_t*)db_start, (const uint32_t*)(ws + L.db_item),
                                 (const unsigned long long*)db_keys, db_order, hdr, behind ? 0 : 1, fill, ipv * V);
          else if (ranked)
              hipLaunchKernelGGL((k_dbin_rank<MGR_DB_RANK_MAX>), dim3((unsigned)(ipv * V + n_fill)), dim3(DBR_THREADS), 0, stream, N, V, ipv, (const uint32_t*)db_start, (const uint32_t*)(ws + L.db_item),
                                 (const unsigned long long*)db_keys, db_order, hdr, behind ? 0 : 1, fill, ipv * V);
          const int fchunk = ranked ? (int)MGR_DB_ITEM : chunk, fchunks = (N + fchunk - 1) / fchunk;
          (void)chunks;
          if (behind)
              hipLaunchKernelGGL((k_dbin_sort<SORT_LDS_KEYS>), dim3(1024 + (ranked ? 0 : n_fill)), dim3(RS_THREADS), SORT_LDS_KEYS * 8 + RS_WAVES * 256 * 4 + 256, stream,
                                 N, fchunk, fchunks, V * fchunks, (const uint32_t*)db_start, (const uint32_t*)db_nvis, db_keys, db_order,
                                 ranked ? cap_keys : 0u, hdr, ranked ? 2 : 0, ranked ? none : fill, 1024); }
        MGR_LAUNCH_CHECK("k_dbin_sort", stream, debug);
        const bool big_possible = T > BIN_SMALL_TILES;
        { MGR_PROF("k_bin_count", stream);
          const dim3 grid_c = (V % 8 == 0) ? dim3(nblk * V) : grid_b;
          hipLaunchKernelGGL((k_bin_count<true>), grid_c, dim3(BCNT_THREADS), (size_t)BIN_SMALL_TILES * 4, stream, N, T, nblk, bb, (const uint32_t*)db_nvis,
                             (const ushort4*)db_bbox, (const uint32_t*)db_order, rect, alive, db_rec, bin_mat, V % 8 == 0 ? 1 : 0);
          if (big_possible && !(skip_tiers & MGR_SKIP_BOX_LARGE))
              hipLaunchKernelGGL((k_bin_count<false>), grid_c, dim3(BCNT_THREADS), (size_t)T * 4, stream, N, T, nblk, bb, (const uint32_t*)db_nvis,
                                 (const ushort4*)db_bbox, (const uint32_t*)db_order, rect, alive, db_rec, bin_mat, V % 8 == 0 ? 1 : 0); }
        { MGR_PROF("k_bin_scan", stream); hipLaunchKernelGGL(k_bin_scan, dim3((T + BSCAN_COLS - 1) / BSCAN_COLS, V), dim3(BSCAN_COLS * BSCAN_SEGS), 0, stream, gx, T, nblk, bb, (const uint32_t*)db_nvis,
                           (const ushort4*)db_bbox, (const uint32_t*)tile_start, bin_mat); }
        { MGR_PROF("k_bin_scatter", stream);
#define MGR_SC_LAUNCH(MK, LDSB, ...)                                                                                                          \
    do {                                                                                                                                  \
        if (spread) hipLaunchKernelGGL((k_bin_scatter<MK, true>), grid_b, dim3(BIN_SC_THREADS), LDSB, stream, __VA_ARGS__);             \
        else hipLaunchKernelGGL((k_bin_scatter<MK, false>), grid_b, dim3(BIN_SC_THREADS), LDSB, stream, __VA_ARGS__);                   \
    } while (0)
          MGR_SC_LAUNCH(BIN_MID_TILES, (size_t)BIN_MID_TILES * 12 + rec_bytes, N, T, nblk, bb,
                             (const uint32_t*)db_nvis, (const ushort4*)db_bbox, (const uint32_t*)db_order, (const uint4*)db_rec, (const uint32_t*)bin_mat,
                             (uint32_t*)(ws + L.sorted_gid), (uint32_t)cap, hdr, skip_tiers);
          if (T > BIN_MID_TILES && !(skip_tiers & MGR_SKIP_BOX_MID))
              MGR_SC_LAUNCH(BIN_SMALL_TILES, (size_t)BIN_SMALL_TILES * 12 + rec_bytes, N, T, nblk, bb,
                            (const uint32_t*)db_nvis, (const ushort4*)db_bbox, (const uint32_t*)db_order, (const uint4*)db_rec, (const uint32_t*)bin_mat,
                            (uint32_t*)(ws + L.sorted_gid), (uint32_t)cap, hdr, 0);
          if (big_possible && !(skip_tiers & MGR_SKIP_BOX_LARGE))
              MGR_SC_LAUNCH(0, (size_t)T * 4 + rec_bytes, N, T, nblk, bb,
                            (const uint32_t*)db_nvis, (const ushort4*)db_bbox, (const uint32_t*)db_order, (const uint4*)db_rec, (const uint32_t*)bin_mat,
                            (uint32_t*)(ws + L.sorted_gid), (uint32_t)cap, hdr, 0);
#undef MGR_SC_LAUNCH
        }
        MGR_LAUNCH_CHECK("k_bin_scatter", stream, debug);
    } else if (N > 0) {
        dim3 grid((N + EMIT_THREADS - 1) / EMIT_THREADS, V);
        { MGR_PROF("k_emit", stream); hipLaunchKernelGGL(k_emit, grid, dim3(EMIT_THREADS), hist_bytes + 16, stream, N, gx, gy,
                           (const float*)(ws + L.depth), (const ushort4*)(ws + L.rect),
                           (const unsigned long long*)(ws + L.alive), tile_start,
                           (uint32_t*)(ws + L.tile_cursor), (unsigned long long*)(ws + L.keys),
                           (uint32_t)cap, lds_hist); }
        MGR_LAUNCH_CHECK("k_emit", stream, debug);
        MgrSideStream& side = mgr_side_stream(device);
        MGR_HIP(side.init());
        MGR_HIP(hipEventRecord(side.fork, stream));
        MGR_HIP(hipStreamWaitEvent(side.stream, side.fork, 0));
        { MGR_PROF("k_tile_split", stream); hipLaunchKernelGGL(k_tile_split, dim3(256), dim3(SORT_THREADS), 0, stream,
                           tile_start, (const uint32_t*)(ws + L.tile_queue), (unsigned long long*)(ws + L.keys),
                           (unsigned long long*)(ws + L.keys2), (uint4*)(ws + L.groups),
                           (uint32_t*)(ws + L.sorted_gid), hdr, (uint32_t)cap); }
        { MGR_PROF("k_tile_sort_small", side.stream); hipLaunchKernelGGL(k_tile_sort_small, dim3(256 * 8), dim3(256), 0, side.stream,
                           tile_start, (const uint32_t*)(ws + L.tile_queue),
                           (const unsigned long long*)(ws + L.keys), (uint32_t*)(ws + L.sorted_gid), hdr,
                           (uint32_t)cap); }
        MGR_HIP(hipEventRecord(side.join, side.stream));
        { MGR_PROF("k_tile_sort", stream); hipLaunchKernelGGL(k_tile_sort, dim3(512), dim3(RS_THREADS), SORT_LDS_KEYS * 8 + RS_WAVES * 256 * 4 + 256, stream,
                           tile_start, (const uint32_t*)(ws + L.tile_queue),
                           (const unsigned long long*)(ws + L.keys), (const unsigned long long*)(ws + L.keys2),
                           (const uint4*)(ws + L.groups), (uint32_t*)(ws + L.sorted_gid), hdr, (uint32_t)cap); }
        MGR_HIP(hipStreamWaitEvent(stream, side.join, 0));
        MGR_LAUNCH_CHECK("k_tile_sort", stream, debug);
    }
    }
    if (!do_blend) return MGR_OK;
    { MGR_PROF("k_blend_fwd", stream); hipLaunchKernelGGL(k_blend_fwd, dim3(MGR_FWD_GRID), dim3(256), 0, stream, N, W, H, gx, gy, VT, bg,
                       (const uint32_t*)(ws + L.tile_queue), (const uint4*)(ws + L.tile_qrec), (const uint32_t*)(ws + L.sorted_gid), (const MgrGRec*)(ws + L.grec), out_color,
                       (uint32_t*)(ws + L.n_contrib), (uint32_t*)(ws + L.tile_done), (uint32_t*)(ws + L.tile_qdone),
                       (float4*)(ws + L.ckpt), hdr, (const uint32_t*)(ws + L.tile_zused), (uint32_t*)(ws + L.tile_qend), bg_filled ? 1 : 0); }
    if (repair && N > 0) {
        { MGR_PROF("k_repair_scan", stream);
          hipLaunchKernelGGL(k_repair_prep, dim3(V), dim3(256), 0, stream, T, gx, hdr, rep_all, (const uint32_t*)(ws + L.tile_zused),
                             (const uint32_t*)(ws + L.tile_zwin));
          hipLaunchKernelGGL(k_repair_scan, dim3(REP_SCAN_SEGS, V), dim3(REP_SCAN_THREADS), 0, stream, N, T, gx, hdr, rep_all, (const int32_t*)radii,
                             (const ushort4*)(ws + L.rect), (const float*)(ws + L.depth), (const MgrGRec*)(ws + L.grec)); }
        { MGR_PROF("k_repair_blend", stream);
          hipLaunchKernelGGL(k_repair_blend, dim3(128), dim3(RS_THREADS), REP_BLEND_LDS, stream, N, W, H, gx, T, hdr, rep_all, bg,
                             (uint32_t*)(ws + L.sorted_gid), (const MgrGRec*)(ws + L.grec), out_color, (uint32_t*)(ws + L.n_contrib),
                             (uint32_t*)(ws + L.tile_qdone), (float4*)(ws + L.ckpt)); }
        MGR_LAUNCH_CHECK("k_repair_blend", stream, debug);
    }
    IlListArgs ll = g_loss_list.take(workspace);
    if (ll.nbx) {
        if (ll.H != H || ll.W != W || ll.list_views != V) return mgr_fail(MGR_EINVAL, "attached loss list: views or image size differ from the forward's");
        ll.tile_start = tile_start;
    }
    const int n_item_blocks = (VT + 255) / 256;
    const MgrFeatStamp stamp = {{(uint32_t)V, (uint32_t)N, (uint32_t)W, (uint32_t)H, (uint32_t)cap}, use_cut ? MGR_FEAT_CUT : 0u};
    { MGR_PROF("k_fwd_items", stream); hipLaunchKernelGGL(k_fwd_items, dim3((unsigned)(n_item_blocks + ll.nbx * V)), dim3(256), 0, stream, (const uint4*)(ws + L.tile_qrec),
                       (const uint32_t*)(ws + L.tile_qdone), (uint32_t*)(ws + L.tile_done), (uint4*)(ws + L.items), hdr,
                       N, T, (const uint32_t*)(ws + L.sorted_gid), (const float*)(ws + L.depth), (const uint32_t*)(ws + L.tile_zused),
                       (const uint32_t*)(ws + L.tile_qend), (uint32_t*)(ws + L.tile_zcut), g_mirror.take(workspace),
                       g_cut_frac, (uint32_t)g_cut_min, g_cut_range, g_cut_rel, gx, g_cut_interior,
                       (const uint32_t*)(ws + L.tile_queue), VT, (unsigned char*)(ws + L.tile_bgok), (const float*)out_color, bg, rep_all,
                       (uint32_t)g_cut_penalty, (uint32_t*)(ws + L.tile_zwin), ll, n_item_blocks, stamp); }
    MGR_LAUNCH_CHECK("k_blend_fwd", stream, debug);
    return MGR_OK;
}

extern "C" int mgr_raster_forward(int V, int N, int W, int H, const float* cams, const float* bg,
                                  const float* means3D, int64_t s_means, const float* cov3D,
                                  int64_t s_cov, const float* colors, int64_t s_col,
                                  const float* opacity, int64_t s_op, float* out_color,
                                  int32_t* radii, void* workspace, size_t workspace_bytes,
                                  int64_t cap, int flags, void* stream_) {
    return raster_forward_impl(V, N, W, H, cams, bg, means3D, s_means, cov3D, s_cov, colors, s_col, opacity, s_op,
                               nullptr, out_color, radii, workspace, workspace_bytes, cap, flags, stream_);
}

extern "C" int mgr_views_forward(int V, int N, int B, int n_articulated, int sh_half, int W, int H, const float* cams, const float* bg,
                                 const float* xyz, const float* log_scale, const float* rot,
                                 const float* opacity_logit, const float* f_dc, const float* f_rest,
                                 const float* skin_w, const float* transforms, float* out_color,
                                 int32_t* radii, void* workspace, size_t workspace_bytes, int64_t cap,
                                 int flags, void* stream_) {
    if (N > 0 && (!xyz || !log_scale || !rot || !opacity_logit || !f_dc || !f_rest || (skin_w && !transforms)))
        return mgr_fail(MGR_EINVAL, "mgr_views_forward: null pointer");
    if (skin_w && (B <= 0 || B > MGR_MAX_BONES)) return mgr_fail(MGR_EINVAL, "mgr_views_forward: bad B");
    if (skin_w && (n_articulated < 0 || n_articulated > N)) return mgr_fail(MGR_EINVAL, "mgr_views_forward: bad n_articulated");
    if (sh_half && ((uintptr_t)f_rest & 15)) return mgr_fail(MGR_EINVAL, "mgr_views_forward: fp16 f_rest must be 16-byte aligned");
    const CanonInputs ci = {B, skin_w ? n_articulated : 0, sh_half ? 1 : 0, xyz, log_scale, rot, opacity_logit, f_dc, f_rest, skin_w, transforms};
    return raster_forward_impl(V, N, W, H, cams, bg, nullptr, 0, nullptr, 0, nullptr, 0, nullptr, 0, &ci, out_color,
                               radii, workspace, workspace_bytes, cap, flags, stream_);
}

#ifdef BIN_PROF
extern "C" int mgr_binprof(unsigned long long* out) {
    MGR_HIP(hipMemcpyFromSymbol(out, HIP_SYMBOL(g_binprof), 8 * 8 * 4096));
    return 0;
}
#endif
extern "C" int mgr_raster_layout(int V, int N, int W, int H, int64_t cap, size_t* out, int n_out) {
    const MgrLayout L = mgr_layout(V, N, W, H, cap);
    const size_t v[] = {L.header, L.grec, L.depth, L.rect, L.alive, L.pair_off, L.tile_count, L.tile_start,
                        L.tile_cursor, L.tile_done, L.tile_queue, L.chunk_start, L.items, L.ckpt, L.keys,
                        L.sorted_gid, L.final_T, L.n_contrib, L.pair_tag, L.pair_grad, L.total, L.inst_grad, L.inst_tag,
                        L.db_nvis, L.db_bbox, L.db_order, L.tile_zcut, L.tile_zused, L.tile_qend, L.tile_rep, L.rep_unit, L.rep_cnt, L.tile_zwin};
    const int n = (int)(sizeof(v) / sizeof(v[0]));
    for (int i = 0; i < n && i < n_out; ++i) out[i] = v[i];
    return n;
}

__global__ void k_debug_pair_alpha(int n, const float* __restrict__ rec, const int32_t* __restrict__ px,
                                   const int32_t* __restrict__ py, float* __restrict__ alpha, int32_t* __restrict__ valid) {
    const int i = blockIdx.x * blockDim.x + threadIdx.x;
    if (i >= n) return;
    float pb[MGR_PAIR_FLOATS];
    const float* r = rec + (size_t)i * 6;
    mgr_pair_store(pb, 0, r[0], r[1], r[2], r[3], r[4], r[5], 0.f, 0.f, 0.f, 1u);
    mgr_pair_pad(pb);
    const float4 R0 = make_float4(pb[0], pb[1], pb[2], pb[3]), R1 = make_float4(pb[4], pb[5], pb[6], pb[7]),
                 R2 = make_float4(pb[8], pb[9], pb[10], pb[11]);
    const mgr_v2f fpx2 = {(float)px[i], (float)px[i]}, fpy2 = {(float)py[i], (float)py[i]};
    mgr_v2f dx, dy, G, al;
    bool va, vb;
    mgr_pair_alpha(R0, R1, R2, fpx2, fpy2, dx, dy, G, al, va, vb);
    alpha[i] = al.x;
    valid[i] = va ? 1 : 0;
}

extern "C" int mgr_debug_pair_alpha(int n, const float* rec, const int32_t* px, const int32_t* py, float* alpha,
                                    int32_t* valid, void* stream_) {
    if (n < 0 || (n > 0 && (!rec || !px || !py || !alpha || !valid))) return mgr_fail(MGR_EINVAL, "mgr_debug_pair_alpha: bad arguments");
    if (n == 0) return MGR_OK;
    hipStream_t stream = (hipStream_t)stream_;
    hipLaunchKernelGGL(k_debug_pair_alpha, dim3((n + 255) / 256), dim3(256), 0, stream, n, rec, px, py, alpha, valid);
    MGR_LAUNCH_CHECK("k_debug_pair_alpha", stream, 0);
    return MGR_OK;
}

static int mgr_overflow_code(uint32_t ovf) {
    if (ovf & MGR_OVF_PAIRS) return mgr_fail(MGR_EOVERFLOW, "pair capacity exceeded");
    if (ovf & MGR_OVF_CUT) return mgr_fail(MGR_ECUT, "depth cut violated: run the forward again without MGR_FWD_DEPTH_CUT");
    if (ovf & MGR_OVF_TIER) return mgr_fail(MGR_ETIER, "a skipped binning launch was needed: run the forward again without MGR_FWD_SKIP_*");
    return MGR_OK;
}

extern "C" int mgr_raster_status_sync(const void* workspace, int64_t* num_pairs, int32_t* overflow,
                                      void* stream_) {
    hipStream_t stream = (hipStream_t)stream_;
    uint32_t h[2] = {0, 0};
    MGR_HIP(hipMemcpyAsync(h, workspace, 8, hipMemcpyDeviceToHost, stream));
    MGR_HIP(hipStreamSynchronize(stream));
    if (num_pairs) *num_pairs = h[0];
    if (overflow) *overflow = (int32_t)h[1];
    return mgr_overflow_code(h[1]);
}

extern "C" int mgr_raster_status_tiers_sync(const void* workspace, int64_t* num_pairs, int32_t* overflow, int32_t* tiers,
                                            void* stream_) {
    hipStream_t stream = (hipStream_t)stream_;
    uint32_t h[64];
    static_assert(offsetof(MgrHeader, sort_near_large) / 4 < 64, "status words beyond the copied part of the header");
    MGR_HIP(hipMemcpyAsync(h, workspace, sizeof(h), hipMemcpyDeviceToHost, stream));
    MGR_HIP(hipStreamSynchronize(stream));
    if (num_pairs) *num_pairs = h[0];
    if (overflow) *overflow = (int32_t)h[1];
    if (tiers) {
        const uint32_t sb = h[offsetof(MgrHeader, sort_big) / 4], sn = h[offsetof(MgrHeader, sort_near_large) / 4], sl = h[offsetof(MgrHeader, sort_large) / 4];
        const uint32_t near_max = MGR_TIERS_NEAR_MASK, beyond_max = MGR_TIERS_BEYOND_SMALL_MASK;
        *tiers = (int32_t)(h[offsetof(MgrHeader, tiers) / 4] | ((sb < near_max ? sb : near_max) << MGR_TIERS_NEAR_SMALL_SHIFT) |
                           ((sn < near_max ? sn : near_max) << MGR_TIERS_NEAR_LARGE_SHIFT) | ((sl < beyond_max ? sl : beyond_max) << MGR_TIERS_BEYOND_SMALL_SHIFT));
    }
    return mgr_overflow_code(h[1]);
}

extern "C" int mgr_raster_debug_binning_sync(const void* workspace, int V, int N, int W, int H,
                                             int64_t cap, int view, int32_t* tile_ranges_host,
                                             int32_t* point_list_host, int64_t max_pairs,
                                             void* stream_) {
    hipStream_t stream = (hipStream_t)stream_;
    const int gx = (W + 15) / 16, gy = (H + 15) / 16, T = gx * gy;
    if (view < 0 || view >= V) return mgr_fail(MGR_EINVAL, "bad view");
    const MgrLayout L = mgr_layout(V, N, W, H, cap);
    const char* ws = (const char*)workspace;
    uint32_t* ts = (uint32_t*)malloc((size_t)(T + 1) * 4);
    MGR_HIP(hipMemcpyAsync(ts, ws + L.tile_start + (size_t)view * T * 4, (size_t)(T + 1) * 4,
                           hipMemcpyDeviceToHost, stream));
    MGR_HIP(hipStreamSynchronize(stream));
    const uint32_t b = ts[0], e = ts[T];
    for (int t = 0; t < T; ++t) {
        tile_ranges_host[2 * t] = (int32_t)(ts[t] - b);
        tile_ranges_host[2 * t + 1] = (int32_t)(ts[t + 1] - b);
    }
    free(ts);
    int64_t n = (int64_t)e - (int64_t)b;
    if (n > max_pairs) n = max_pairs;
    if (n > 0 && point_list_host) {
        MGR_HIP(hipMemcpyAsync(point_list_host, ws + L.sorted_gid + (size_t)b * 4, (size_t)n * 4,
                               hipMemcpyDeviceToHost, stream));
        MGR_HIP(hipStreamSynchronize(stream));
    }
    return MGR_OK;
}
```

### manus_amd/engine.py

```python
import ctypes
import functools
import os

import numpy as np
import torch
import torch.distributed as dist

from . import fused as fused_mod, losses, ops, rasterizer
from . import _lib
from ._lib import ManusHipError, check, lib, ptr, stream

GRAD_LAYOUT = (("_xyz", 3), ("_features_dc", 3), ("_features_rest", 45), ("_opacity", 1),
               ("_scaling", 3), ("_rotation", 4))
GRAD_WIDTH = sum(w for _, w in GRAD_LAYOUT)
FLAT_TAIL = 2

LAYOUT_TILE_START, LAYOUT_TILE_DONE = 7, 9
LAYOUT_FINAL_T, LAYOUT_N_CONTRIB, LAYOUT_INST_TAG = 16, 17, 22
LAYOUT_TILE_ZCUT, LAYOUT_TILE_ZUSED, LAYOUT_TILE_QEND = 26, 27, 28
LAYOUT_TILE_REP, LAYOUT_REP_UNIT, LAYOUT_REP_CNT, LAYOUT_TILE_ZWIN = 29, 30, 31, 32


def flat_size(N):
    return N * (GRAD_WIDTH + 2) + FLAT_TAIL
# ... 739 lines not shown
        key = (V, N, W, H, ws.cap)
        off = self._ts_off.get(key)
        if off is None:
            arr = (ctypes.c_size_t * 40)()
            lib().mgr_raster_layout(V, N, W, H, ws.cap, arr, 40)
            off = self._ts_off[key] = [int(x) for x in arr]
        return off

    def _target_map(self, view_ids, sel, bg):
        m = sel.get("tmap")
        if m is None:
            H, W = int(self.s["height"]), int(self.s["width"])
            per = int(lib().mgr_image_loss_target_map_words(1, H, W))
            rows = []
            for k, v in enumerate(view_ids):
                t = self._tmaps.get(v)
                if t is None:
                    t = torch.empty(per, dtype=torch.int32, device=self.device)
                    check(lib().mgr_image_loss_target_map(1, H, W, ptr(sel["targets"][k]), ptr(bg), ptr(t), stream()),
                          "mgr_image_loss_target_map")
                    while len(self._tmaps) >= self.MAX_TARGET_MAPS:
                        self._tmaps.pop(next(iter(self._tmaps)))
                    self._tmaps[v] = t
                rows.append(t)
            m = sel["tmap"] = torch.stack(rows).contiguous()
        return m

    def _tile_start_ptr(self, ws, V, N, W, H):
        return ws.buf.data_ptr() + self._layout(ws, V, N, W, H)[LAYOUT_TILE_START]

    def _cut_flag(self, ws, view_ids, V, N, W, H):
        ctx = self.rz.context(self.device)
        if not self.depth_cut or not ctx.fenced(self.sync_check):
            return 0
        lay = self._layout(ws, V, N, W, H)
        T = ((W + 15) // 16) * ((H + 15) // 16)
        return self._cut.flag(ws, view_ids, ctx.cut_retries, (lay[LAYOUT_TILE_ZCUT], lay[LAYOUT_TILE_ZWIN]), 4 * V * T,
                              self.cut_repair, self.cut_margin, self.cut_penalty)

    def _step_direct(self, view_ids, scale, g_img=None):
        s, p = self.s, {k: v.detach() for k, v in self.params.items()}
        sel = self._select(view_ids)
        dev = self.device
        N, na, V = p["_xyz"].shape[0], self.n_art, len(view_ids)
        W, H = int(s["width"]), int(s["height"])
        kept = self._kept if (self.persistent_grads and not self.grad_arena and self.fused) else None
        if kept is not None:
            kept.begin(N, na, dev)
        map_on = self._map_terms()
        w, B = self._skin_weights(p["_xyz"], na)
        if kept is not None:
            out = kept.get((V, 3, H, W), ("image", V, H, W), zeroed=False)
        else:
            out = torch.empty((V, 3, H, W), dtype=torch.float32, device=dev)
        radii = torch.empty((V, N), dtype=torch.int32, device=dev)
        f_rest, sh_half = self._sh_storage(p["_features_rest"])
        head = (V, N, B, na, sh_half, W, H, ptr(sel["cams"]), ptr(s["bg"]), ptr(p["_xyz"]), ptr(p["_scaling"]), ptr(p["_rotation"]),
                ptr(p["_opacity"].reshape(-1)), ptr(p["_features_dc"]), ptr(f_rest), ptr(w), ptr(sel["T"]))
        fwd = (head, out, radii, kept)
        self._loss_ssim = None
        self.last_corrected = None
        E = self._exposure_table() if g_img is None else None
        listed = g_img is None and E is None and self.loss == "l1+ssim" and self.sparse_loss and self._ssim_mode() == "rows"
        route = None if not listed else "mapped" if self.target_map else "overlap" if self.overlap_loss else None
        loss_list = self._mapped_loss_list(view_ids, sel, V, H, W) if route == "mapped" else None
        ctx = self.rz.context(dev)
        ws = None
        try:
            ws, _ = ctx.forward(V, N, W, H, self._forward_launch(fwd, view_ids, loss_list, _lib.MGR_FWD_NO_BLEND if route == "overlap" else 0),
                                sync_check=self.sync_check, defer_fence=True)
            if route != "overlap" and ctx.fenced(self.sync_check):
                ctx.fence(ws)
            given = g_img is not None
            d_E = None
            if E is not None:
                loss, g_img, lp, d_E = self._exposure_loss(out, E, sel, view_ids, scale)
            else:
                loss, g_img = self._loss(ctx, ws, fwd, sel, scale, g_img, route, loss_list)
                lp = None if given else self._lpips_term(out, sel["targets"], scale, g_img, sel, view_ids)
            grads, d_w, st_g, st_v, st_r, d_T = self._backward(ws, fwd, g_img, scale, full_rows=any(map_on))
            map_out = self._map_chain(ws, head, sel, view_ids, scale, map_on, grads, d_w, d_T) if any(map_on) else None
            active = self._skin_backward(ws, head, p["_xyz"], d_w, grads["_xyz"], full_rows=any(map_on))
            d_grid = self._skin_grid_backward(head, p["_xyz"], d_w, active, rows_of_d_w=any(map_on)) if self.skin_grid_grad else None
            overflow = ws.buf[4:8].view(torch.int32)
        except BaseException:
            self._lws.pop((V, H, W), None)
            self._kept.invalidate()
            raise
        finally:
            if ws is not None:
                ws.busy = False
        self.last_image, self.last_radii = out, radii
        self.last_active = active
        res = dict(grads=grads, grad2d=st_g, vis=st_v, radii=st_r, loss=loss, overflow=overflow)
        if map_out is not None:
            res["loss"] = loss + map_out[0]
            res["loss_mask"], res["loss_depth"] = map_out[1], map_out[2]
        if lp is not None:
            res["loss"] = res["loss"] + self.w_lpips * lp
            res["loss_lpips"] = lp
        if self._loss_ssim is not None:
            res["loss_ssim"] = self._loss_ssim
        if d_T is not None:
            res["d_transforms"] = d_T
        if d_E is not None:
            res["d_exposure"] = d_E
        if d_grid is not None:
            res["d_skin_grid"] = d_grid
        return res

    def _skin_weights(self, xyz, na):
        if not na:
            return None, 0
        s, sg = self.s, self.grid
        w = torch.empty((na, sg.B), dtype=torch.float32, device=self.device)
        check(lib().mgr_skin_weights_fwd(na, ptr(xyz), ptr(sg.data), sg.D, sg.H, sg.W, sg.B, sg.stride,
                                         ptr(s["grid_center"]), ptr(s["grid_scale"]), ptr(w), stream()),
              "mgr_skin_weights_fwd")
        return w, sg.B

    def _mapped_loss_list(self, view_ids, sel, V, H, W):
        nbytes = int(lib().mgr_image_loss_workspace_bytes(V, H, W))
        lws = self._lws.get((V, H, W))
        if lws is None:
            lws = self._lws[(V, H, W)] = torch.zeros(nbytes, dtype=torch.uint8, device=self.device)
        return lws, self._target_map(view_ids, sel, self.s["bg"]), nbytes

    def _views_forward(self, ws, fwd, phase):
        head, out, radii, kept = fwd
        bits = phase | self._cut.bit | ws.skip_bits() | (_lib.MGR_FWD_IMAGE_KEPT if (kept is not None and kept.image_ws is ws) else 0)
        check(lib().mgr_views_forward(*head, ptr(out), ptr(radii), ptr(ws.buf), ws.nbytes, ws.cap, bits, stream()), "mgr_views_forward")
        if kept is not None:
            kept.image_ws = ws

    def _forward_launch(self, fwd, view_ids, loss_list, phase):
        V, N, W, H = fwd[0][0], fwd[0][1], fwd[0][5], fwd[0][6]
        launches = [0]

        def launch(ws):
            self._cut.bit = self._cut_flag(ws, view_ids, V, N, W, H)
            if loss_list is None or not self.attach_list:
                return self._views_forward(ws, fwd, phase)
            lws, tmap, nbytes = loss_list
            if launches[0]:
                lws.zero_()
            launches[0] += 1
            check(lib().mgr_views_forward_attach_loss_list(ptr(ws.buf), V, H, W, ptr(tmap), ptr(lws), nbytes),
                  "mgr_views_forward_attach_loss_list")
            try:
                self._views_forward(ws, fwd, 0)
            except Exception:
                lib().mgr_views_forward_attach_loss_list(ptr(ws.buf), V, H, W, None, None, 0)
                raise

        return launch

    def _loss(self, ctx, ws, fwd, sel, scale, g_img, route, loss_list):
        head, out = fwd[0], fwd[1]
        V, N, W, H = head[0], head[1], head[5], head[6]
        tgt, bg = sel["targets"], self.s["bg"]
        if route is None:
            if g_img is not None:
                return (out * g_img).sum(), g_img.contiguous()
            return self._image_loss(out, tgt, scale, tiles=(bg, self._tile_start_ptr(ws, V, N, W, H)))
        if route == "mapped":
            lws, tmap, nbytes = loss_list
            if not self.attach_list:
                check(lib().mgr_image_loss_tiles_list_mapped(V, H, W, ptr(tmap), ptr(bg), ctypes.c_void_p(self._tile_start_ptr(ws, V, N, W, H)),
                                                             ptr(lws), nbytes, 1, stream()), "mgr_image_loss_tiles_list_mapped")
        else:
            nbytes = int(lib().mgr_image_loss_workspace_bytes(V, H, W))
            lws = torch.empty(nbytes, dtype=torch.uint8, device=self.device)
            cur = torch.cuda.current_stream(self.device)
            if self._side is None:
                self._side = torch.cuda.Stream(device=self.device)
            self._side.wait_stream(cur)
            with torch.cuda.stream(self._side):
                check(lib().mgr_image_loss_tiles_list(V, H, W, ptr(tgt), ptr(bg), ctypes.c_void_p(self._tile_start_ptr(ws, V, N, W, H)),
                                                      ptr(lws), nbytes, stream()), "mgr_image_loss_tiles_list")
            self._views_forward(ws, fwd, _lib.MGR_FWD_BLEND_ONLY)
            if ctx.fenced(self.sync_check):
                ctx.fence(ws)
            cur.wait_stream(self._side)
            lws.record_stream(self._side)
        k, const = self._loss_scales(out, scale)
        g_img = torch.empty_like(out)
        sums = torch.empty(3, dtype=torch.float32, device=self.device)
        check(lib().mgr_image_loss_tiles_finish(V, H, W, ptr(out), ptr(tgt), self.w_rgb, self.w_ssim, k, const, ptr(g_img),
                                                ptr(sums), ptr(lws), nbytes, stream()), "mgr_image_loss_tiles_finish")
        return sums[2], g_img

    def _map_chain(self, ws, head, sel, view_ids, scale, map_on, grads, d_w, d_T=None):
        V, N, B, na, _, W, H = head[:7]
        cams, xyz, ls, rot, op, w, T = head[7], head[9], head[10], head[11], head[12], head[15], head[16]
        dev, L = self.device, lib()
        masks, depths = self._map_sel(sel, view_ids, map_on[1])
        key = (V, N, W, H, ws.cap, bool(map_on[1]))
        mb = self._map_bufs.get(key)
        if mb is None:
            e = functools.partial(torch.empty, dtype=torch.float32, device=dev)
            n_loss, n_scr = int(L.mgr_map_loss_workspace_bytes(V, H, W)), int(L.mgr_views_maps_backward_workspace_bytes(V, N, W, H, ws.cap))
            mb = dict(alpha=e((V, H, W)), g_alpha=e((V, H, W)), depth=e((V, 1, H, W)) if map_on[1] else None,
                      g_depth=e((V, 1, H, W)) if map_on[1] else None,
                      loss_ws=torch.empty(n_loss, dtype=torch.uint8, device=dev), scratch=torch.empty(n_scr, dtype=torch.uint8, device=dev))
            self._map_bufs = {key: mb}
        sums = torch.empty(3, dtype=torch.float32, device=dev)
        rc = L.mgr_raster_blend_features(V, N, 0, W, H, None, 0, None, int(map_on[1]), ptr(mb["depth"]), ptr(mb["alpha"]), ptr(ws.buf),
                                         ws.nbytes, ws.cap, stream())
        if rc == _lib.MGR_ESTATE and int(ws.buf[4:8].view(torch.int32).item()) != 0:
            z = torch.zeros((), dtype=torch.float32, device=dev)
            return z, z, z
        check(rc, "mgr_raster_blend_features")
        k = scale * V
        check(L.mgr_map_loss(V, H, W, ptr(mb["alpha"]), ptr(masks), ptr(mb["depth"]), ptr(depths), self.w_mask,
                             self.w_depth if map_on[1] else 0.0, k, ptr(mb["g_alpha"]), ptr(mb["g_depth"]), ptr(sums), ptr(mb["loss_ws"]),
                             mb["loss_ws"].numel(), stream()), "mgr_map_loss")
        args = (V, N, B, na, W, H, cams, xyz, ls, rot, op, w, T, ptr(mb["alpha"]), ptr(mb["depth"]), ptr(mb["g_alpha"]), ptr(mb["g_depth"]), 1,
                ptr(grads["_xyz"]), ptr(grads["_scaling"]), ptr(grads["_rotation"]), ptr(grads["_opacity"]), ptr(d_w), ptr(ws.buf),
                ws.nbytes, ws.cap, ptr(mb["scratch"]), mb["scratch"].numel(), 0)
        if d_T is not None:
            nbytes = int(L.mgr_views_maps_pose_workspace_bytes(V, N, B))
            if self._map_pose_ws is None or self._map_pose_ws.numel() < nbytes:
# ... 530 lines not shown
```

### manus_amd/rasterizer.py

```python
from typing import NamedTuple

import ctypes
import os
import time
import weakref

import torch
import torch.nn as nn

from . import _lib
from ._lib import (check, f32c, lib, ptr, stream, MGR_FWD_RANK_LARGE, MGR_FWD_SKIP_BOX_LARGE, MGR_FWD_SKIP_BOX_MID, MGR_FWD_SKIP_SORT_BEHIND,
                   MGR_FWD_SPREAD, MGR_OVF_CUT, MGR_OVF_FLAGS_MASK, MGR_OVF_PAIRS, MGR_OVF_REPAIRED_SHIFT, MGR_OVF_TIER, MGR_TIERS_BEYOND_SMALL_MASK,
                   MGR_TIERS_BEYOND_SMALL_SHIFT, MGR_TIERS_BOX_LARGE, MGR_TIERS_BOX_MID, MGR_TIERS_NEAR_LARGE_SHIFT, MGR_TIERS_NEAR_MASK,
                   MGR_TIERS_NEAR_SMALL_SHIFT, MGR_TIERS_WIDE_RECT)
from .ops import lbs_cov, sh_colors


class GaussianRasterizationSettings(NamedTuple):
    image_height: int
    image_width: int
    tanfovx: float
    tanfovy: float
    bg: torch.Tensor
    scale_modifier: float
    viewmatrix: torch.Tensor
    projmatrix: torch.Tensor
    sh_degree: int
    campos: torch.Tensor
    prefiltered: bool
    debug: bool


class RasterWorkspace:
    SORT_BIG_MAX = int(os.environ.get("MANUS_SORT_BIG_MAX", "0"))

    def __init__(self, device, V, N, W, H, cap):
        self.key = (V, N, W, H)
        self.cap = int(cap)
        self.nbytes = int(lib().mgr_raster_workspace_bytes(V, N, W, H, self.cap))
        self.buf = torch.zeros(self.nbytes, dtype=torch.uint8, device=device)
        self.busy = False
        self.hint_key = self.prev_hint_key = None
        self.cut_block = False
        self.mirror = None
        self.tiers = None
        self.no_flagging_skips = False

    def skip_bits(self):
        t = self.tiers
        if t is None:
            return 0
        large = (t >> MGR_TIERS_BEYOND_SMALL_SHIFT) & MGR_TIERS_BEYOND_SMALL_MASK
        near = (t >> (MGR_TIERS_NEAR_LARGE_SHIFT if large else MGR_TIERS_NEAR_SMALL_SHIFT)) & MGR_TIERS_NEAR_MASK
        bits = ((MGR_FWD_RANK_LARGE if large else 0) | (MGR_FWD_SPREAD if t & MGR_TIERS_WIDE_RECT else 0))
        if not self.no_flagging_skips:
            bits |= ((0 if t & MGR_TIERS_BOX_LARGE else MGR_FWD_SKIP_BOX_LARGE) | (0 if t & MGR_TIERS_BOX_MID else MGR_FWD_SKIP_BOX_MID)
                     | (MGR_FWD_SKIP_SORT_BEHIND if near <= RasterWorkspace.SORT_BIG_MAX else 0))
        return bits


def default_pair_capacity(V, N):
    return max(4096, 8 * V * max(N, 1))


class RasterContext:

    MAX_FENCES = 64
    AUTO_FENCE_AFTER = int(os.environ.get("MANUS_AUTO_FENCE_AFTER", "8"))

    def __init__(self, device):
        self.device = torch.device(device)
        self.pool = {}
        self.cap_hint = {}
        self.sync_every_forward = True
        self.last_ws = None
        self._fences = []
        self._free_pinned = []
        self._evicted_overflow = False
        self.cut_retries = 0
        self.cut_repairs = 0
        self._clean = {}
        self._seen = {}
        self.auto_fenced = 0
        self.tier_retries = 0

    def acquire(self, V, N, W, H, min_cap):
        lst = self.pool.setdefault((V, N, W, H), [])
        for ws in lst:
            if not ws.busy and ws.cap >= min_cap:
                ws.busy = True
                return ws
        lst[:] = [w for w in lst if w.busy]
        ws = RasterWorkspace(self.device, V, N, W, H, min_cap)
        ws.busy = True
        lst.append(ws)
        return ws

    def clear(self):
        if self._fences:
            torch.cuda.synchronize(self.device)
        for ws, pinned, ev in self._fences:
            if pinned is not None:
                self._free_pinned.append(pinned)
        for lst in self.pool.values():
            for ws in lst:
                if ws.mirror is not None:
                    lib().mgr_raster_set_status_mirror(ptr(ws.buf), None)
                    self._free_pinned.append(ws.mirror)
                    ws.mirror = None
        self.pool.clear()
        self.cap_hint.clear()
        self._fences.clear()
        self._evicted_overflow = False
        self.last_ws = None
        self._clean.clear()
        self._seen.clear()

    _SYNC = (False, MGR_OVF_PAIRS, MGR_OVF_PAIRS | MGR_OVF_CUT)
    _FENCE = (True, 0, 0)
    _RECHECK = (True, MGR_OVF_PAIRS, 0)

    def _read_header(self, ws):
        npairs, ovf, tiers = ctypes.c_int64(0), ctypes.c_int32(0), ctypes.c_int32(0)
        rc = lib().mgr_raster_status_tiers_sync(ptr(ws.buf), ctypes.byref(npairs), ctypes.byref(ovf), ctypes.byref(tiers), stream())
        return rc, int(npairs.value), int(ovf.value), int(tiers.value)

    def _digest(self, ws, npairs, word, tiers, route):
        learn_flagged, cut_hidden_by, tier_hidden_by = route
        ovf = word & MGR_OVF_FLAGS_MASK
        self.cut_repairs += word >> MGR_OVF_REPAIRED_SHIFT
        if learn_flagged or not ovf:
            self.cap_hint[ws.key] = max(self.cap_hint.get(ws.key, 0), int(npairs * 1.25) + 4096)
        ws.tiers = None if ovf & MGR_OVF_TIER else tiers
        if ovf & MGR_OVF_CUT and not ovf & cut_hidden_by:
            ws.cut_block = True
            self.cut_retries += 1
        if ovf & MGR_OVF_TIER and not ovf & tier_hidden_by:
            self.tier_retries += 1
        return ovf

    def _seen_cams(self, key, cams):
        ent = self._seen.get(key, {}).get(id(cams))
        return ent is not None and ent[0]() is cams and ent[1] == cams._version

    def _see_cams(self, key, cams):
        seen = self._seen.setdefault(key, {})
        if len(seen) >= 256:
            seen.clear()
        seen[id(cams)] = (weakref.ref(cams), cams._version)

    def forward(self, V, N, W, H, launch, sync_check=True, defer_fence=False, auto_fence=False, cams=None):
        key = (V, N, W, H)
        cap = max(self.cap_hint.get(key, 0), default_pair_capacity(V, N))
        auto = (bool(auto_fence) and sync_check and self.sync_every_forward and 0 < self.AUTO_FENCE_AFTER <= self._clean.get(key, 0)
                and cams is not None and self._seen_cams(key, cams))
        if auto:
            try:
                self.poll()
            except _lib.ManusHipError:
                self._clean[key] = 0
                raise _lib.ManusHipError("an unsynchronised forward of the previous step outgrew its pair capacity: its image and "
                                         "gradients were incomplete.  The capacity was enlarged and this context reads the pair count "
                                         "back again; set MANUS_AUTO_FENCE_AFTER=0 to keep every forward synchronous.")
        while True:
            ws = self.acquire(V, N, W, H, cap)
            ws.prev_hint_key, ws.hint_key = ws.hint_key, None
            fenced = auto or not (sync_check and self.sync_every_forward)
            ws.no_flagging_skips = auto
            if fenced:
                self._arm_mirror(ws)
            launch(ws)
            self.last_ws = ws
            if fenced:
                if auto:
                    self.auto_fenced += 1
                if not defer_fence:
                    self._fence(ws)
                return ws, None
            rc, npairs, word, tiers = self._read_header(ws)
            self._digest(ws, npairs, word, tiers, self._SYNC)
            if rc == _lib.MGR_OK:
                self._clean[key] = self._clean.get(key, 0) + 1
                if auto_fence and cams is not None:
                    self._see_cams(key, cams)
                return ws, npairs
            self._clean[key] = 0
# ... 389 lines not shown
```

Before: 770.6.

## Run k_fwd_items and loss fold on a side stream, move loss list into bin count

Moves the k_fwd_items kernel and, in phase 2, the image-loss fold kernel onto a side stream, so they overlap with later work on the main stream. Event-based pending joins are keyed by workspace and inserted at every consumer: backward, the state readbacks, the next forward and workspace eviction. The attached loss-list workgroups move from k_fwd_items to extra blocks on the k_bin_count launch, with a standalone fallback kernel. This trades extra event record and wait calls, plus a mutex-protected pending table, for the chance of overlapping small kernels, and a missed join could cause a race.

Result: no change. 766.4 (-0.5%).

```diff
diff --git a/include/manus_hip.h b/include/manus_hip.h
--- a/include/manus_hip.h
+++ b/include/manus_hip.h
@@ -341,6 +341,7 @@
 int mgr_image_loss_tiles_finish(int V, int H, int W, const float* pred, const float* target, float w_l1, float w_ssim,
                                 float grad_scale, float loss_offset, float* dL_dpred, float* sums, void* workspace,
                                 size_t workspace_bytes, void* stream);
+int mgr_side_stream_join(const void* workspace, void* stream);
 
 #define MGR_IL2D_DENSE 1
 size_t mgr_image_loss2d_workspace_bytes(int V, int H, int W);
diff --git a/manus_amd/_lib.py b/manus_amd/_lib.py
--- a/manus_amd/_lib.py
+++ b/manus_amd/_lib.py
@@ -72,6 +72,7 @@
     "mgr_raster_layout": (c_int, [c_int, c_int, c_int, c_int, c_i64, ctypes.POINTER(c_sz), c_int]),
     "mgr_raster_status_sync": (c_int, [c_vp, ctypes.POINTER(c_i64), ctypes.POINTER(ctypes.c_int32), c_vp]),
     "mgr_raster_set_status_mirror": (c_int, [c_vp, c_vp]),
+    "mgr_side_stream_join": (c_int, [c_vp, c_vp]),
     "mgr_raster_set_cut_margin": (c_int, [c_f32, c_int, c_f32, c_f32, c_int]),
     "mgr_raster_set_cut_penalty": (c_int, [c_int]),
     "mgr_raster_status_tiers_sync": (c_int, [c_vp, ctypes.POINTER(c_i64), ctypes.POINTER(ctypes.c_int32),
diff --git a/manus_amd/csrc/image_loss.hip b/manus_amd/csrc/image_loss.hip
--- a/manus_amd/csrc/image_loss.hip
+++ b/manus_amd/csrc/image_loss.hip
@@ -418,6 +418,7 @@
     if (workspace_bytes < mgr_image_loss_workspace_bytes(V, H, W))
         return mgr_fail(MGR_ENOMEM, "mgr_image_loss: workspace too small");
     hipStream_t stream = (hipStream_t)stream_;
+    MGR_HIP(mgr_side_join(workspace, stream));
     IlWindow win;
     float sum = 0.f;
     for (int i = 0; i < 11; ++i) {
@@ -461,8 +462,12 @@
                            grad_scale, dL_dpred, partial, (const uint32_t*)work_list, (const uint32_t*)work_count,
                            (int)grid.x, (int)grid.y, acc_slots, (uint32_t)nb, sum_lim, work_count + 1);
     }
-    hipLaunchKernelGGL(k_image_loss_fold, dim3(1), dim3(IL_ACC_SLOTS), 0, stream, acc_slots, (long long)V * H * W * 3,
+    hipStream_t fold_stream = stream;
+    const bool aside = phase == 2 && mgr_side_on(MGR_SIDE_FOLD);
+    if (aside) MGR_HIP(mgr_side_fork(stream, &fold_stream));
+    hipLaunchKernelGGL(k_image_loss_fold, dim3(1), dim3(IL_ACC_SLOTS), 0, fold_stream, acc_slots, (long long)V * H * W * 3,
                        sums, grad_scale * w_l1, -grad_scale * w_ssim, loss_offset, work_count);
+    if (aside) MGR_HIP(mgr_side_pend(workspace, fold_stream, stream));
     MGR_LAUNCH_CHECK("k_image_loss", stream, 0);
     return MGR_OK;
 }
diff --git a/manus_amd/csrc/mgr_common.h b/manus_amd/csrc/mgr_common.h
--- a/manus_amd/csrc/mgr_common.h
+++ b/manus_amd/csrc/mgr_common.h
@@ -46,6 +46,13 @@
     }
 };
 #define MGR_PROF(name, stream) MgrProfScope mgr_prof_scope_(name, stream)
+
+#define MGR_SIDE_ITEMS 0
+#define MGR_SIDE_FOLD 1
+bool mgr_side_on(int what);
+hipError_t mgr_side_fork(hipStream_t stream, hipStream_t* side);
+hipError_t mgr_side_pend(const void* key, hipStream_t side, hipStream_t stream);
+hipError_t mgr_side_join(const void* key, hipStream_t stream);
 
 #define MGR_WHY_UNITS 1u
 #define MGR_WHY_VIEW_TILES 2u
diff --git a/manus_amd/csrc/raster_bwd.hip b/manus_amd/csrc/raster_bwd.hip
--- a/manus_amd/csrc/raster_bwd.hip
+++ b/manus_amd/csrc/raster_bwd.hip
@@ -1089,6 +1089,7 @@
         return mgr_fail(MGR_EINVAL, "mgr_raster_backward: bad sizes");
     if (!cams || !bg || !dL_dcolor || !out_color || !workspace)
         return mgr_fail(MGR_EINVAL, "mgr_raster_backward: null pointer");
+    MGR_HIP(mgr_side_join(workspace, stream));
     if (N == 0) return MGR_OK;
     if (!canon && (!means3D || !cov3D || !dL_dmeans3D || !dL_dmeans2D || !dL_dcolors || !dL_dopacity || !dL_dcov3D))
         return mgr_fail(MGR_EINVAL, "mgr_raster_backward: null pointer");
diff --git a/manus_amd/csrc/raster_feat.hip b/manus_amd/csrc/raster_feat.hip
--- a/manus_amd/csrc/raster_feat.hip
+++ b/manus_amd/csrc/raster_feat.hip
@@ -165,6 +165,7 @@
 static int feat_read_state(const char* who, const char* ws, const MgrLayout& L, int V, int N, int W, int H, int64_t cap, int VT,
                            hipStream_t stream, MgrHeader& h) {
     const size_t head_bytes = offsetof(MgrHeader, qctr);
+    MGR_HIP(mgr_side_join(ws, stream));
     MGR_HIP(hipMemcpyAsync(&h, ws + L.header, head_bytes, hipMemcpyDeviceToHost, stream));
     MGR_HIP(hipStreamSynchronize(stream));
     if (h.fwd_seq == 0u) return mgr_fail(MGR_ESTATE, "%s: no forward has run on this workspace", who);
@@ -185,6 +186,7 @@
 extern "C" int mgr_raster_forward_seq_sync(const void* workspace, uint32_t* seq, void* stream_) {
     hipStream_t stream = (hipStream_t)stream_;
     if (!workspace || !seq) return mgr_fail(MGR_EINVAL, "mgr_raster_forward_seq_sync: null pointer");
+    MGR_HIP(mgr_side_join(workspace, stream));
     MGR_HIP(hipMemcpyAsync(seq, (const char*)workspace + offsetof(MgrHeader, fwd_seq), 4, hipMemcpyDeviceToHost, stream));
     MGR_HIP(hipStreamSynchronize(stream));
     return MGR_OK;
diff --git a/manus_amd/csrc/raster_fwd.hip b/manus_amd/csrc/raster_fwd.hip
--- a/manus_amd/csrc/raster_fwd.hip
+++ b/manus_amd/csrc/raster_fwd.hip
@@ -1378,9 +1378,16 @@
                                                             const uint32_t* __restrict__ db_order,
                                                             const ushort4* __restrict__ rect,
                                                             const unsigned long long* __restrict__ alive,
-                                                            uint4* __restrict__ db_rec, uint32_t* __restrict__ bin_mat, int xcd_order) {
+                                                            uint4* __restrict__ db_rec, uint32_t* __restrict__ bin_mat, int xcd_order,
+                                                            const IlListArgs ll, int n_bin_x) {
     extern __shared__ uint32_t s_mem[];
     uint32_t* s_hist = s_mem;
+    if (SMALL && (int)blockIdx.x >= n_bin_x) {
+        const int lb = (int)blockIdx.x - n_bin_x;
+        if (xcd_order) il_list_mapped_block(ll, lb % ll.nbx, lb / ll.nbx, s_mem);
+        else il_list_mapped_block(ll, lb, (int)blockIdx.y, s_mem);
+        return;
+    }
     const int tid = threadIdx.x;
     int v = blockIdx.y, b = blockIdx.x;
     if (xcd_order) {
@@ -2521,13 +2528,8 @@
                                                    float cut_range, float cut_rel, int gx, int interior_only,
                                                    const uint32_t* __restrict__ tile_queue, int VT, unsigned char* __restrict__ tile_bgok,
                                                    const float* out_color, const float* __restrict__ bg, const MgrRep rep, uint32_t cut_penalty,
-                                                   uint32_t* __restrict__ tile_zwin, const IlListArgs ll, int n_item_blocks, const MgrFeatStamp stamp) {
+                                                   uint32_t* __restrict__ tile_zwin, int n_item_blocks, const MgrFeatStamp stamp) {
     __shared__ uint32_t s_scan[8];
-    if ((int)blockIdx.x >= n_item_blocks) {
-        const int lb = (int)blockIdx.x - n_item_blocks;
-        il_list_mapped_block(ll, lb % ll.nbx, lb / ll.nbx, s_scan);
-        return;
-    }
     __shared__ uint32_t s_base;
     __shared__ uint32_t s_run[257];
     __shared__ uint4 s_qr[256], s_qd[256], s_rp[256];
@@ -2637,6 +2639,11 @@
     }
 }
 
+__global__ __launch_bounds__(ILS_T) void k_fwd_loss_list(const IlListArgs ll) {
+    __shared__ uint32_t s2[2];
+    il_list_mapped_block(ll, (int)blockIdx.x, (int)blockIdx.y, s2);
+}
+
 struct CanonInputs {
     int B, n_art, sh_half;
     const float *xyz, *log_scale, *rot, *op_logit, *f_dc, *f_rest, *skin_w, *transforms;
@@ -2658,6 +2665,74 @@
 static MgrSideStream& mgr_side_stream(int device) {
     static thread_local MgrSideStream s[MGR_MAX_DEVICES];
     return s[device];
+}
+
+static std::mutex g_pend_mu;
+static struct { const void* key; hipEvent_t ev; int device; bool pending; } g_pend[64];
+
+bool mgr_side_on(int what) {
+    const char* e = getenv("MANUS_SIDE_STREAM");
+    if (!e || !e[0] || e[0] == '1') return true;
+    if (e[0] == '0') return false;
+    return e[0] == (what == MGR_SIDE_ITEMS ? 'i' : 'f');
+}
+
+hipError_t mgr_side_fork(hipStream_t stream, hipStream_t* side_out) {
+    int device = 0;
+    hipError_t e = hipGetDevice(&device);
+    if (e != hipSuccess) return e;
+    if (device < 0 || device >= MGR_MAX_DEVICES) return hipErrorInvalidDevice;
+    MgrSideStream& side = mgr_side_stream(device);
+    if ((e = side.init()) != hipSuccess) return e;
+    if ((e = hipEventRecord(side.fork, stream)) != hipSuccess) return e;
+    if ((e = hipStreamWaitEvent(side.stream, side.fork, 0)) != hipSuccess) return e;
+    *side_out = side.stream;
+    return hipSuccess;
+}
+
+hipError_t mgr_side_pend(const void* key, hipStream_t side, hipStream_t stream) {
+    int device = 0;
+    hipError_t e = hipGetDevice(&device);
+    if (e != hipSuccess) return e;
+    std::lock_guard<std::mutex> lk(g_pend_mu);
+    int k_use = -1;
+    for (int k = 0; k < 64; ++k) {
+        if (g_pend[k].pending && g_pend[k].key == key) { k_use = k; break; }
+        if (!g_pend[k].pending && k_use < 0) k_use = k;
+    }
+    if (k_use < 0) {
+        MgrSideStream& s = mgr_side_stream(device);
+        if ((e = hipEventRecord(s.join, side)) != hipSuccess) return e;
+        return hipStreamWaitEvent(stream, s.join, 0);
+    }
+    auto& p = g_pend[k_use];
+    if (p.ev && p.device != device) { (void)hipEventDestroy(p.ev); p.ev = nullptr; }
+    if (!p.ev && (e = hipEventCreateWithFlags(&p.ev, hipEventDisableTiming)) != hipSuccess) return e;
+    p.device = device;
+    if ((e = hipEventRecord(p.ev, side)) != hipSuccess) return e;
+    p.key = key; p.pending = true;
+    return hipSuccess;
+}
+
+hipError_t mgr_side_join(const void* key, hipStream_t stream) {
+    int device = 0;
+    if (!key) {
+        const hipError_t e = hipGetDevice(&device);
+        if (e != hipSuccess) return e;
+    }
+    std::lock_guard<std::mutex> lk(g_pend_mu);
+    for (auto& p : g_pend) {
+        if (!p.pending || (key ? p.key != key : p.device != device)) continue;
+        const hipError_t e = hipStreamWaitEvent(stream, p.ev, 0);
+        if (e != hipSuccess) return e;
+        p.pending = false;
+    }
+    return hipSuccess;
+}
+
+extern "C" int mgr_side_stream_join(const void* workspace, void* stream_) {
+    MGR_HIP(mgr_side_join(workspace, (hipStream_t)stream_));
+    return MGR_OK;
 }
 
 static std::mutex g_slot_mu;
@@ -2768,6 +2843,14 @@
         MGR_HIP(hipFuncSetAttribute((const void*)k_bin_scatter<0, true>, hipFuncAttributeMaxDynamicSharedMemorySize, 152 * 1024));
         MGR_HIP(hipFuncSetAttribute((const void*)k_repair_blend, hipFuncAttributeMaxDynamicSharedMemorySize, REP_BLEND_LDS));
         attr_set[device].store(true, std::memory_order_release);
+    }
+
+    MGR_HIP(mgr_side_join(workspace, stream));
+    IlListArgs ll = do_blend ? g_loss_list.take(workspace) : IlListArgs();
+    if (ll.nbx) {
+        if (ll.H != H || ll.W != W || ll.list_views != V) return mgr_fail(MGR_EINVAL, "attached loss list: views or image size differ from the forward's");
+        ll.tile_start = tile_start;
+        MGR_HIP(mgr_side_join(ll.partial, stream));
     }
 
     const int lds_hist = ((size_t)T * 4 + 128 <= 150 * 1024) ? 1 : 0;
@@ -2865,11 +2948,13 @@
         const bool big_possible = T > BIN_SMALL_TILES;
         { MGR_PROF("k_bin_count", stream);
           const dim3 grid_c = (V % 8 == 0) ? dim3(nblk * V) : grid_b;
-          hipLaunchKernelGGL((k_bin_count<true>), grid_c, dim3(BCNT_THREADS), (size_t)BIN_SMALL_TILES * 4, stream, N, T, nblk, bb, (const uint32_t*)db_nvis,
-                             (const ushort4*)db_bbox, (const uint32_t*)db_order, rect, alive, db_rec, bin_mat, V % 8 == 0 ? 1 : 0);
+          const dim3 grid_l = (V % 8 == 0) ? dim3((unsigned)(nblk * V + ll.nbx * V)) : dim3((unsigned)(nblk + ll.nbx), V);
+          hipLaunchKernelGGL((k_bin_count<true>), grid_l, dim3(BCNT_THREADS), (size_t)BIN_SMALL_TILES * 4, stream, N, T, nblk, bb, (const uint32_t*)db_nvis,
+                             (const ushort4*)db_bbox, (const uint32_t*)db_order, rect, alive, db_rec, bin_mat, V % 8 == 0 ? 1 : 0, ll, (int)grid_c.x);
+          ll.nbx = 0;
           if (big_possible && !(skip_tiers & MGR_SKIP_BOX_LARGE))
               hipLaunchKernelGGL((k_bin_count<false>), grid_c, dim3(BCNT_THREADS), (size_t)T * 4, stream, N, T, nblk, bb, (const uint32_t*)db_nvis,
-                                 (const ushort4*)db_bbox, (const uint32_t*)db_order, rect, alive, db_rec, bin_mat, V % 8 == 0 ? 1 : 0); }
+                                 (const ushort4*)db_bbox, (const uint32_t*)db_order, rect, alive, db_rec, bin_mat, V % 8 == 0 ? 1 : 0, IlListArgs(), (int)grid_c.x); }
         { MGR_PROF("k_bin_scan", stream); hipLaunchKernelGGL(k_bin_scan, dim3((T + BSCAN_COLS - 1) / BSCAN_COLS, V), dim3(BSCAN_COLS * BSCAN_SEGS), 0, stream, gx, T, nblk, bb, (const uint32_t*)db_nvis,
                            (const ushort4*)db_bbox, (const uint32_t*)tile_start, bin_mat); }
         { MGR_PROF("k_bin_scatter", stream);
@@ -2922,6 +3007,11 @@
     }
     }
     if (!do_blend) return MGR_OK;
+    static_assert(BCNT_THREADS == ILS_T, "the span list's workgroups ride on k_bin_count's launch");
+    if (ll.nbx) {
+        MGR_PROF("k_fwd_loss_list", stream);
+        hipLaunchKernelGGL(k_fwd_loss_list, dim3((unsigned)ll.nbx, V), dim3(ILS_T), 0, stream, ll);
+    }
     { MGR_PROF("k_blend_fwd", stream); hipLaunchKernelGGL(k_blend_fwd, dim3(MGR_FWD_GRID), dim3(256), 0, stream, N, W, H, gx, gy, VT, bg,
                        (const uint32_t*)(ws + L.tile_queue), (const uint4*)(ws + L.tile_qrec), (const uint32_t*)(ws + L.sorted_gid), (const MgrGRec*)(ws + L.grec), out_color,
                        (uint32_t*)(ws + L.n_contrib), (uint32_t*)(ws + L.tile_done), (uint32_t*)(ws + L.tile_qdone),
@@ -2938,21 +3028,20 @@
                              (uint32_t*)(ws + L.tile_qdone), (float4*)(ws + L.ckpt)); }
         MGR_LAUNCH_CHECK("k_repair_blend", stream, debug);
     }
-    IlListArgs ll = g_loss_list.take(workspace);
-    if (ll.nbx) {
-        if (ll.H != H || ll.W != W || ll.list_views != V) return mgr_fail(MGR_EINVAL, "attached loss list: views or image size differ from the forward's");
-        ll.tile_start = tile_start;
-    }
     const int n_item_blocks = (VT + 255) / 256;
     const MgrFeatStamp stamp = {{(uint32_t)V, (uint32_t)N, (uint32_t)W, (uint32_t)H, (uint32_t)cap}, use_cut ? MGR_FEAT_CUT : 0u};
-    { MGR_PROF("k_fwd_items", stream); hipLaunchKernelGGL(k_fwd_items, dim3((unsigned)(n_item_blocks + ll.nbx * V)), dim3(256), 0, stream, (const uint4*)(ws + L.tile_qrec),
+    const bool aside = mgr_side_on(MGR_SIDE_ITEMS) && !repair && !debug;
+    hipStream_t caller = stream;
+    if (aside) MGR_HIP(mgr_side_fork(caller, &stream));
+    { MGR_PROF("k_fwd_items", stream); hipLaunchKernelGGL(k_fwd_items, dim3((unsigned)n_item_blocks), dim3(256), 0, stream, (const uint4*)(ws + L.tile_qrec),
                        (const uint32_t*)(ws + L.tile_qdone), (uint32_t*)(ws + L.tile_done), (uint4*)(ws + L.items), hdr,
                        N, T, (const uint32_t*)(ws + L.sorted_gid), (const float*)(ws + L.depth), (const uint32_t*)(ws + L.tile_zused),
                        (const uint32_t*)(ws + L.tile_qend), (uint32_t*)(ws + L.tile_zcut), g_mirror.take(workspace),
                        g_cut_frac, (uint32_t)g_cut_min, g_cut_range, g_cut_rel, gx, g_cut_interior,
                        (const uint32_t*)(ws + L.tile_queue), VT, (unsigned char*)(ws + L.tile_bgok), (const float*)out_color, bg, rep_all,
-                       (uint32_t)g_cut_penalty, (uint32_t*)(ws + L.tile_zwin), ll, n_item_blocks, stamp); }
-    MGR_LAUNCH_CHECK("k_blend_fwd", stream, debug);
+                       (uint32_t)g_cut_penalty, (uint32_t*)(ws + L.tile_zwin), n_item_blocks, stamp); }
+    if (aside) MGR_HIP(mgr_side_pend(workspace, stream, caller));
+    MGR_LAUNCH_CHECK("k_blend_fwd", caller, debug);
     return MGR_OK;
 }
 
@@ -3038,6 +3127,7 @@
                                       void* stream_) {
     hipStream_t stream = (hipStream_t)stream_;
     uint32_t h[2] = {0, 0};
+    MGR_HIP(mgr_side_join(workspace, stream));
     MGR_HIP(hipMemcpyAsync(h, workspace, 8, hipMemcpyDeviceToHost, stream));
     MGR_HIP(hipStreamSynchronize(stream));
     if (num_pairs) *num_pairs = h[0];
@@ -3050,6 +3140,7 @@
     hipStream_t stream = (hipStream_t)stream_;
     uint32_t h[64];
     static_assert(offsetof(MgrHeader, sort_near_large) / 4 < 64, "status words beyond the copied part of the header");
+    MGR_HIP(mgr_side_join(workspace, stream));
     MGR_HIP(hipMemcpyAsync(h, workspace, sizeof(h), hipMemcpyDeviceToHost, stream));
     MGR_HIP(hipStreamSynchronize(stream));
     if (num_pairs) *num_pairs = h[0];
@@ -3072,6 +3163,7 @@
     if (view < 0 || view >= V) return mgr_fail(MGR_EINVAL, "bad view");
     const MgrLayout L = mgr_layout(V, N, W, H, cap);
     const char* ws = (const char*)workspace;
+    MGR_HIP(mgr_side_join(workspace, stream));
     uint32_t* ts = (uint32_t*)malloc((size_t)(T + 1) * 4);
     MGR_HIP(hipMemcpyAsync(ts, ws + L.tile_start + (size_t)view * T * 4, (size_t)(T + 1) * 4,
                            hipMemcpyDeviceToHost, stream));
diff --git a/manus_amd/engine.py b/manus_amd/engine.py
--- a/manus_amd/engine.py
+++ b/manus_amd/engine.py
@@ -845,10 +845,12 @@
             map_out = self._map_chain(ws, head, sel, view_ids, scale, map_on, grads, d_w, d_T) if any(map_on) else None
             active = self._skin_backward(ws, head, p["_xyz"], d_w, grads["_xyz"], full_rows=any(map_on))
             d_grid = self._skin_grid_backward(head, p["_xyz"], d_w, active, rows_of_d_w=any(map_on)) if self.skin_grid_grad else None
+            check(lib().mgr_side_stream_join(None, stream()), "mgr_side_stream_join")
             overflow = ws.buf[4:8].view(torch.int32)
         except BaseException:
             self._lws.pop((V, H, W), None)
             self._kept.invalidate()
+            lib().mgr_side_stream_join(None, stream())
             raise
         finally:
             if ws is not None:
@@ -901,6 +903,8 @@
         launches = [0]
 
         def launch(ws):
+            if self.depth_cut:
+                check(lib().mgr_side_stream_join(ptr(ws.buf), stream()), "mgr_side_stream_join")
             self._cut.bit = self._cut_flag(ws, view_ids, V, N, W, H)
             if loss_list is None or not self.attach_list:
                 return self._views_forward(ws, fwd, phase)
diff --git a/manus_amd/rasterizer.py b/manus_amd/rasterizer.py
--- a/manus_amd/rasterizer.py
+++ b/manus_amd/rasterizer.py
@@ -90,6 +90,8 @@
             if not ws.busy and ws.cap >= min_cap:
                 ws.busy = True
                 return ws
+        if any(not w.busy for w in lst):
+            lib().mgr_side_stream_join(None, stream())
         lst[:] = [w for w in lst if w.busy]
         ws = RasterWorkspace(self.device, V, N, W, H, min_cap)
         ws.busy = True
@@ -102,6 +104,8 @@
         for ws, pinned, ev in self._fences:
             if pinned is not None:
                 self._free_pinned.append(pinned)
+        if self.pool:
+            lib().mgr_side_stream_join(None, stream())
         for lst in self.pool.values():
             for ws in lst:
                 if ws.mirror is not None:
```
